# dariopagliaricci/Metal-PathTracer-arm64

Measured on AMD Instinct MI355X. Metric: Msamples/sec (whole node) at 1920×1080, depth 8; PFM RMSE vs Embree ref, higher is better.
Workload: dtype f32; 1 GPU; BASELINE configs[1]: Cornell box + one 70,688-triangle OBJ mesh, 1920x1080, depth 8, 256 spp, seed 1337; partition=8-row bands round-robin over 1 rank(s), RCCL gather of the HDR buffer

## Files before the change

### metal-pathtracer-arm64_amd/__init__.py

```python
from __future__ import annotations

import ctypes as C
import os
from typing import Optional, Tuple

import numpy as np

_PKG_DIR = os.path.dirname(os.path.abspath(__file__))
LIB_PATH = os.path.join(_PKG_DIR, "libptr_hip.so")
CLI_PATH = os.path.join(_PKG_DIR, "PathTracerHeadless")



class PtrSphere(C.Structure):
    _fields_ = [("centerRadius", C.c_float * 4), ("materialIndex", C.c_uint32 * 4)]


class PtrRect(C.Structure):
    _fields_ = [
        ("corner", C.c_float * 4),
        ("edgeU", C.c_float * 4),
        ("edgeV", C.c_float * 4),
        ("normalAndPlane", C.c_float * 4),
        ("materialTwoSided", C.c_uint32 * 4),
# ... 346 lines not shown
class PtrFrameInfo(C.Structure):
    _fields_ = [
        ("width", C.c_uint32),
        ("height", C.c_uint32),
        ("minCount", C.c_uint32),
        ("maxCount", C.c_uint32),
        ("totalSamples", C.c_uint64),
        ("uniform", C.c_uint32),
        ("reserved", C.c_uint32),
    ]


_frame_info = C.POINTER(PtrFrameInfo)
_FRAME_SIGNATURES = {
    "ptr_frame_create": (_int, [_vp, _settings, C.POINTER(_vp)] + _err),
    "ptr_frame_release": (None, [_vp]),
    "ptr_frame_reset": (_int, [_vp, _settings] + _err),
    "ptr_frame_accumulate": (_int, [_vp, _u32, _vp, _stats] + _err),
    "ptr_frame_refine": (_int, [_vp, _adaptive, _vp, _stats, _adaptive_info] + _err),
    "ptr_frame_resolve_device": (_int, [_vp, _vp, _vp, _vp, _vp] + _err),
    "ptr_frame_resolve": (_int, [_vp, _fp, _fp, _up] + _err),
    "ptr_frame_info": (_int, [_vp, _frame_info]),
    "ptr_frame_export": (_int, [_vp, _fp, _fp, _fp, _up, _fp] + _err),
    "ptr_frame_import": (_int, [_vp, _fp, _fp, _fp, _up, _fp] + _err),
    "ptr_frame_debug_create": (_int, [_u32, _u32, _fp, _u32, _int, C.POINTER(_vp)] + _err),
}
FRAME_SYMBOLS = tuple(_FRAME_SIGNATURES)

_MULTI_FRAME_SIGNATURES = {
    "ptr_multi_frame_create": (_int, [_desc, _settings, _int, C.POINTER(_vp)] + _err),
    "ptr_multi_frame_release": (None, [_vp]),
    "ptr_multi_frame_reset": (_int, [_vp, _settings] + _err),
    "ptr_multi_frame_accumulate": (_int, [_vp, _u32, _stats] + _err),
    "ptr_multi_frame_refine": (_int, [_vp, _adaptive, _stats, _adaptive_info] + _err),
    "ptr_multi_frame_resolve": (_int, [_vp, _fp, _fp, _up, _fp, _fp] + _err),
    "ptr_multi_frame_resolve_device": (_int, [_vp, _vp, _vp, _vp, _vp] + _err),
    "ptr_multi_frame_info": (_int, [_vp, _frame_info, _multi_info]),
    "ptr_multi_frame_export": (_int, [_vp, _fp, _fp, _fp, _up, _fp] + _err),
    "ptr_multi_frame_import": (_int, [_vp, _fp, _fp, _fp, _up, _fp] + _err),
    "ptr_multi_frame_debug_create_on": (_int, [_desc, _settings, _ids, _int, C.POINTER(_vp)] + _err),
    "ptr_multi_frame_debug_create": (_int, [_u32, _u32, _fp, _u32, _ids, _int, C.POINTER(_vp)] + _err),
}
MULTI_FRAME_SYMBOLS = tuple(_MULTI_FRAME_SIGNATURES)



class PtrMeshTransform(C.Structure):
    _fields_ = [("meshIndex", C.c_uint32), ("pad", C.c_uint32), ("localToWorld", C.c_float * 16)]


class PtrUpdateInfo(C.Structure):
    _fields_ = [
        ("totalSeconds", C.c_double),
        ("bakeMs", C.c_double),
        ("refitMs", C.c_double),
        ("quantiseMs", C.c_double),
        ("wideMs", C.c_double),
        ("trianglesMoved", C.c_uint64),
        ("nodes", C.c_uint64),
        ("levels", C.c_uint64),
        ("wideNodes", C.c_uint64),
        ("sceneLo", C.c_float * 3),
        ("sceneHi", C.c_float * 3),
        ("gridOrigin", C.c_float * 3),
        ("gridCell", C.c_float * 3),
        ("cellOverExtent", C.c_float),
        ("pad", C.c_uint32),
    ]

    def as_dict(self) -> dict:
        return {name: (list(getattr(self, name)) if hasattr(getattr(self, name), "__len__") else getattr(self, name))
                for name, _ in self._fields_ if name != "pad"}


_DYNAMIC_SIGNATURES = {
    "ptr_scene_upload_dynamic": (_int, [_desc, _int, C.POINTER(_vp)] + _err),
    "ptr_scene_set_mesh_transforms": (_int, [_vp, C.POINTER(PtrMeshTransform), _u32, _vp, C.POINTER(PtrUpdateInfo)] + _err),
    "ptr_scene_is_dynamic": (_int, [_vp]),
    "ptr_debug_scene_arrays": (_int, [_vp, _u32, _vp, _u64, _u64p]),
    "ptr_debug_dynamic_tables": (_int, [_desc, _u32, _vp, _u64, _u64p] + _err),
}
DYNAMIC_SYMBOLS = tuple(_DYNAMIC_SIGNATURES)

SCENE_ARRAYS = {"tris": (0, np.float32, (3, 4)), "triNormals": (1, np.float32, (3, 4)), "triUv": (2, np.float32, (4, 4)),
                "triTangent": (3, np.float32, (3, 4)), "triBounds": (4, np.float32, (2, 4)), "sphereBounds": (5, np.float32, (2, 4)),
                "boxes": (6, np.float32, (4, 4)), "qnodes": (7, np.uint32, (2, 4)), "wnodes": (8, np.uint32, (4, 4)), "grid": (9, np.float32, (3,))}
DYNAMIC_TABLES = {"nodes": (0, np.float32, (4, 4)), "qnodes": (1, np.uint32, (2, 4)), "wnodes": (2, np.uint32, (4, 4)),
                  "triBounds": (3, np.float32, (2, 4)), "sphereBounds": (4, np.float32, (2, 4)), "schedule": (5, np.uint32, ()),
                  "levelOffsets": (6, np.uint32, ()), "wideSource": (7, np.uint32, (4,)), "grid": (8, np.float32, (3,)),
                  "requantised": (9, np.uint32, (2, 4)), "meshTriOffsets": (10, np.uint32, ()), "meshTris": (11, np.uint32, ()),
                  "info": (12, np.uint32, ())}
DYNAMIC_TABLE_INFO = ("nodes", "levels", "wide_nodes", "quantized", "triangles", "spheres", "max_depth", "root_ref", "oversize_ref", "wide_depth")

_lib: Optional[C.CDLL] = None


class PtrError(RuntimeError):
    pass


def load_library() -> C.CDLL:
    global _lib
    if _lib is not None:
        return _lib
    path = os.environ.get("PTR_HIP_LIBRARY", LIB_PATH)
    if not os.path.exists(path):
        raise PtrError(f"{path} is missing: run `python -c 'import __graft_entry__ as g; g.build()'` first")
    lib = C.CDLL(path)
    for name, (restype, argtypes) in list(_SIGNATURES.items()) + list(_POST_SIGNATURES.items()) + list(_STATS_SIGNATURES.items()) + \
            list(_ADAPTIVE_SIGNATURES.items()) + list(_MULTI_SIGNATURES.items()) + list(_FRAME_SIGNATURES.items()) + list(_MULTI_FRAME_SIGNATURES.items()) + \
            list(_DYNAMIC_SIGNATURES.items()):
        fn = getattr(lib, name)
        fn.restype, fn.argtypes = restype, argtypes
    _lib = lib
    return lib


def _err_buf():
    return C.create_string_buffer(1024)


def _check(rc: int, err) -> None:
    if rc != 0:
        raise PtrError(err.value.decode("utf-8", "replace") or f"libptr_hip call failed ({rc})")


def _fptr(a: np.ndarray):
    return a.ctypes.data_as(C.POINTER(C.c_float))


def _uptr(a: np.ndarray):
    return a.ctypes.data_as(C.POINTER(C.c_uint32))


def _batch(fn, lead, inp, dtype, cols, outs, more=(), tail=()):
    ptr = lambda a: _uptr(a) if a.dtype == np.uint32 else _fptr(a)
    inp = np.ascontiguousarray(inp, dtype=dtype).reshape(-1, cols)
    res = [np.zeros((inp.shape[0],) + shape, dtype=dt) for shape, dt in outs]
    err = _err_buf()
    _check(fn(*lead, ptr(inp), *more, inp.shape[0], *map(ptr, res), *tail, err, len(err)), err)
    return res[0] if len(res) == 1 else tuple(res)


def device_count() -> int:
    return int(load_library().ptr_device_count())


BAND_ROWS = 8


def band_count(height: int, part: int = 0, parts: int = 1) -> int:
    return int(load_library().ptr_part_band_count(height, part, parts))




class HostScene:

    def __init__(self, handle: C.c_void_p):
        self._h = handle
        self.desc = PtrSceneDesc()
        self.settings = PtrSettings()
        load_library().ptr_host_scene_desc(self._h, C.byref(self.desc), C.byref(self.settings))

    @classmethod
    def load(cls, scene_path: str, asset_dir: Optional[str] = None) -> "HostScene":
        lib = load_library()
        h = C.c_void_p()
        err = _err_buf()
        rc = lib.ptr_host_scene_load(os.fsencode(scene_path), os.fsencode(asset_dir) if asset_dir else None,
                                     C.byref(h), err, len(err))
        _check(rc, err)
        return cls(h)

    def settings_for(self, width: Optional[int] = None, height: Optional[int] = None, max_depth: Optional[int] = None,
                     seed: Optional[int] = None, **overrides) -> PtrSettings:
        s = self.settings.copy()
        if width:
            s.width = width
        if height:
            s.height = height
        if max_depth is not None:
            s.maxDepth = max_depth
        if seed is not None:
            s.seed = seed
        for k, v in overrides.items():
            setattr(s, k, v)
        if s.width == 0:
            s.width = 1280
        if s.height == 0:
            s.height = 720
        return s

    def close(self) -> None:
# ... 677 lines not shown
    err = _err_buf()
    _check(lib.ptr_host_write_exr_multilayer(os.fsencode(path), _fptr(rgb), w, h, _fptr(counts) if counts is not None else None,
                                             colorspace.encode(), err, len(err)), err)


def read_pfm(path: str) -> np.ndarray:
    lib = load_library()
    w, h = C.c_uint32(), C.c_uint32()
    if lib.ptr_host_read_pfm(os.fsencode(path), None, 0, C.byref(w), C.byref(h)) != 0:
        raise PtrError(f"cannot read PFM header: {path}")
    out = np.zeros((h.value, w.value, 3), dtype=np.float32)
    if lib.ptr_host_read_pfm(os.fsencode(path), _fptr(out), out.size, C.byref(w), C.byref(h)) != 0:
        raise PtrError(f"cannot read PFM data: {path}")
    return out




def debug_eval_bsdf(material: PtrMaterial, settings: PtrSettings, inputs: np.ndarray) -> np.ndarray:
    return _batch(load_library().ptr_debug_eval_bsdf, (C.byref(material), C.byref(settings)), inputs, np.float32, 12, [((5,), np.float32)])


def debug_sample_bsdf(material: PtrMaterial, settings: PtrSettings, inputs: np.ndarray, front: np.ndarray,
                      states: np.ndarray):
    front = np.ascontiguousarray(front, dtype=np.uint32)
    states = np.ascontiguousarray(states, dtype=np.uint32)
    return _batch(load_library().ptr_debug_sample_bsdf, (C.byref(material), C.byref(settings)), inputs, np.float32, 9,
                  [((8,), np.float32), ((), np.uint32)], more=(_uptr(front), _uptr(states)))


def debug_sample_lobes(material: PtrMaterial, settings: PtrSettings, inputs: np.ndarray, front: np.ndarray, states: np.ndarray):
    front = np.ascontiguousarray(front, dtype=np.uint32)
    states = np.ascontiguousarray(states, dtype=np.uint32)
    env_rough = C.c_float()
    out, sample, out_states = _batch(load_library().ptr_debug_sample_lobes, (C.byref(material), C.byref(settings)), inputs, np.float32, 9,
                                     [((3,), np.float32), ((8,), np.float32), ((), np.uint32)], more=(_uptr(front), _uptr(states)),
                                     tail=(C.byref(env_rough),))
    return out, sample, out_states, float(env_rough.value)


def debug_env_mips(rgba: np.ndarray):
    rgba = np.ascontiguousarray(rgba, dtype=np.float32)
    h, w = rgba.shape[0], rgba.shape[1]
    lib = load_library()
    levels = C.c_uint32(0)
    if lib.ptr_debug_env_mips(_fptr(rgba), w, h, None, 0, C.byref(levels)) != 0:
        raise PtrError("ptr_debug_env_mips failed")
    sizes = [(max(h >> l, 1), max(w >> l, 1)) for l in range(levels.value)]
    out = np.zeros(sum(a * b for a, b in sizes) * 4, dtype=np.float32)
    if lib.ptr_debug_env_mips(_fptr(rgba), w, h, _fptr(out), out.size, C.byref(levels)) != 0:
        raise PtrError("ptr_debug_env_mips failed")
    chain, at = [], 0
    for a, b in sizes:
        chain.append(out[at:at + a * b * 4].reshape(a, b, 4))
        at += a * b * 4
    return chain


def debug_camera_rays(settings: PtrSettings, xys: np.ndarray):
    return _batch(load_library().ptr_debug_camera_rays, (C.byref(settings),), xys, np.uint32, 3, [((6,), np.float32), ((), np.uint32)])


def debug_env_distribution(rgba: np.ndarray) -> dict:
    rgba = np.ascontiguousarray(rgba, dtype=np.float32)
    h, w = rgba.shape[0], rgba.shape[1]
    pdf = np.zeros((h, w), np.float32)
    ca = np.zeros((h, w), np.uint32)
    ct = np.zeros((h, w), np.float32)
    ma = np.zeros(h, np.uint32)
    mt = np.zeros(h, np.float32)
    total = C.c_float()
    rc = load_library().ptr_debug_env_distribution(_fptr(rgba), w, h, _fptr(pdf), _uptr(ca), _fptr(ct), _uptr(ma), _fptr(mt),
                                                   C.byref(total))
    if rc != 0:
        raise PtrError("environment map has no positive radiance")
    return dict(pdf=pdf, cond_alias=ca, cond_threshold=ct, marg_alias=ma, marg_threshold=mt, total=total.value)


GEOMETRY_FIELDS = ("nodes", "leaves", "triangles_referenced", "spheres_referenced", "max_depth", "max_leaf_size",
                   "unreferenced", "multiply_referenced", "box_violations", "quant_violations", "bad_refs", "triangles",
                   "spheres", "sah_cost_milli", "build_ms", "quantized_usable")


def debug_scene_geometry(desc: PtrSceneDesc, leaf_max: int = 0) -> dict:
    out = (C.c_uint64 * 16)()
    err = _err_buf()
    _check(load_library().ptr_debug_scene_geometry(C.byref(desc), leaf_max, out, err, len(err)), err)
    g = dict(zip(GEOMETRY_FIELDS, [int(v) for v in out]))
    word = g["quantized_usable"]
    g["oversize"] = (word >> 8) & 0xFF
    g["wide_nodes"] = (word >> 16) & 0xFFFFFFFF
    g["wide_depth"] = (word >> 48) & 0xFF
    g["wide_problems"] = word >> 63
    g["quantized_usable"] = word & 0xFF
    return g


def debug_dynamic_tables(desc: PtrSceneDesc, names=None) -> dict:
    lib = load_library()
    out = {}
    for name in (names or DYNAMIC_TABLES):
        which, dtype, shape = DYNAMIC_TABLES[name]
        size = C.c_uint64(0)
        err = _err_buf()
        _check(lib.ptr_debug_dynamic_tables(C.byref(desc), which, None, 0, C.byref(size), err, len(err)), err)
        buf = np.zeros(size.value // np.dtype(dtype).itemsize, dtype)
        _check(lib.ptr_debug_dynamic_tables(C.byref(desc), which, buf.ctypes.data_as(C.c_void_p), buf.nbytes, C.byref(size), err, len(err)), err)
        out[name] = buf.reshape(2, 3) if name == "grid" else buf.reshape((-1,) + shape)
    if "info" in out:
        out["info"] = dict(zip(DYNAMIC_TABLE_INFO, (int(v) for v in out["info"])))
    return out


def walk_stack_depths(desc: PtrSceneDesc, rays: np.ndarray) -> np.ndarray:
    return _batch(load_library().ptr_debug_walk_stack_depths, (C.byref(desc),), rays, np.float32, 8, [((), np.uint32)])
```

### metal-pathtracer-arm64_amd/csrc/host/debug_probes.cpp

```cpp
#include <algorithm>
#include <cmath>

#include "device_scene.h"
#include "ptr_debug.h"

using namespace ptrk;
using namespace ptrhost;

namespace {

bool checkProbeRays(const float* rays, uint64_t n, bool infiniteTmax, const char* who, char* err, size_t err_cap) {
    if (n >= (1ull << kConnectMaskShift)) {
        setErr(err, err_cap, std::string(who) + ": at most 2^27 - 1 rays");
        return false;
    }
    for (uint64_t i = 0; i < n; ++i) {
        const float tmin = rays[i * 8 + 3], tmax = rays[i * 8 + 7];
        if (tmin != 1.0e-4f || (infiniteTmax && !(std::isinf(tmax) && tmax > 0.0f))) {
            setErr(err, err_cap, std::string(who) + ": ray " + std::to_string(i) + " has tmin " + std::to_string(tmin) + " / tmax " +
                                     std::to_string(tmax) + (infiniteTmax ? "; the kernel traces from 1e-4 to infinity" : "; the kernel traces from 1e-4"));
            return false;
        }
    }
    return true;
}

void probeInfo(const PtrDeviceScene& ds, bool count, uint32_t info[4]) {
    info[0] = static_cast<uint32_t>(traversalNodeFormat(ds.view, count));
    info[1] = ds.view.stackLimit;
    info[2] = ds.view.useWide ? ds.wideDepth : 0u;
    info[3] = kLdsStackLevels;
}

LaunchConfig probeLaunchConfig(const PtrDeviceScene& ds) {
    LaunchConfig cfg = coldLaunchConfig(ds);
    cfg.feederChunk = ds.feederChunk;
    HIP_CHECK(hipMemset(cfg.workCounters, 0, 2 * sizeof(uint32_t)));
    return cfg;
}

struct BsdfProbe {
    DeviceBuffer<float4> material;
    RenderParams rp;
    BsdfProbe(const PtrMaterial& m, const PtrSettings& settings) {
        std::vector<float> rows;
        compactMaterial(m, rows);
        material.upload(reinterpret_cast<const float4*>(rows.data()), kMaterialVec4);
        fillRenderParams(settings, 1, rp);
    }
};

}

extern "C" {

int ptr_debug_render_signatures(PtrDeviceScene* scene, const PtrSettings* settings, float* out_rgb, uint32_t* out_signature, char* err,
                                size_t err_cap) {
    return deviceCall("ptr_debug_render_signatures", scene, scene && settings && out_signature, err, err_cap, [&] {
        const size_t pixels = static_cast<size_t>(settings->width) * settings->height;
        const size_t floats = static_cast<size_t>(ptr_part_band_count(settings->height, 0, 1)) * PTR_BAND_ROWS * settings->width * 3u;
        scene->outBands.ensure(floats);
        PtrRenderStats stats{};
        renderBands(*scene, *settings, 1u, 0u, 1u, scene->outBands.ptr, nullptr, 1, &stats);
        if (out_rgb) scene->outBands.download(out_rgb, pixels * 3u);
        std::vector<float4> items(pixels);
        std::vector<uint32_t> pixelOfLocal(pixels);
        scene->itemAccum.download(items.data(), pixels);
        scene->pixelOfLocal.download(pixelOfLocal.data(), pixels);
        for (size_t lp = 0; lp < pixels; ++lp) {
            uint32_t bits;
            std::memcpy(&bits, &items[lp].w, sizeof(bits));
            out_signature[pixelOfLocal[lp]] = bits;
        }
    });
}

int ptr_debug_texture_sample(PtrDeviceScene* scene, uint32_t texture, const float* in, uint64_t n, float* out, char* err, size_t err_cap) {
    return deviceCall("ptr_debug_texture_sample", scene, scene && (in || !n) && (out || !n), err, err_cap, [&] {
        if (n == 0) return;
        DeviceBuffer<float> din;
        DeviceBuffer<float4> dout;
        din.upload(in, n * 3);
        dout.ensure(n);
        launchDebugTexSample(scene->view, texture, din.ptr, n, dout.ptr, nullptr);
        dout.download(reinterpret_cast<float4*>(out), n);
    });
// ... 69 lines not shown
            HIP_CHECK(hipMemset(scene->counters.ptr, 0, sizeof(uint64_t) * kCounterSlots));
            pool.counters = scene->counters.ptr;
        }
        launchExtend(scene->view, pool, probeLaunchConfig(*scene), nullptr, count != 0, nullptr);
        HIP_CHECK(hipGetLastError());
        launchDebugHitRecords(scene->view, dRays.ptr, dHit.ptr, n, static_cast<uint32_t>(scene->info[2]), static_cast<uint32_t>(scene->info[3]),
                              dOut.ptr, nullptr);
        HIP_CHECK(hipDeviceSynchronize());
        dOut.download(out, n);
    });
}

int ptr_debug_connect_rays(PtrDeviceScene* scene, const float* rays, const uint32_t* ignore_light, uint64_t n, uint32_t records_per_slot,
                           uint32_t* occluded, uint32_t info[4], char* err, size_t err_cap) {
    const bool argsOk = scene && (rays || !n) && (occluded || !n) && info;
    if (argsOk && (records_per_slot < 1u || records_per_slot > 4u)) {
        setErr(err, err_cap, "ptr_debug_connect_rays: records_per_slot must be 1..4");
        return 1;
    }
    if (argsOk && !checkProbeRays(rays, n, false, "ptr_debug_connect_rays", err, err_cap)) return 1;
    for (uint64_t i = 0; argsOk && ignore_light && i < n; ++i) {
        if (ignore_light[i] != 0xFFFFFFFFu && ignore_light[i] >= scene->view.rectLightCount) {
            setErr(err, err_cap, "ptr_debug_connect_rays: ray " + std::to_string(i) + " ignores light " + std::to_string(ignore_light[i]) +
                                     " of " + std::to_string(scene->view.rectLightCount));
            return 1;
        }
    }
    return deviceCall("ptr_debug_connect_rays", scene, argsOk, err, err_cap, [&] {
        probeInfo(*scene, false, info);
        if (n == 0) return;
        std::vector<float4> lights(static_cast<size_t>(scene->view.rectLightCount) * kRectLightVec4);
        scene->rectLights.download(lights.data(), lights.size());
        const uint64_t slots = (n + records_per_slot - 1u) / records_per_slot;
        std::vector<float4> rec(slots * kRecSlots * 4u, make_float4(0.0f, 0.0f, 0.0f, 0.0f));
        for (uint64_t i = 0; i < n; ++i) {
            const float* r = rays + i * 8;
            const uint64_t slot = i / records_per_slot, k = i % records_per_slot;
            const uint32_t light = ignore_light ? ignore_light[i] : 0xFFFFFFFFu;
            const uint32_t kind = light == 0xFFFFFFFFu ? 0u : 3u;
            rec[(k * 4u + 0u) * slots + slot] = make_float4(r[0], r[1], r[2], r[7]);
            rec[(k * 4u + 1u) * slots + slot] = make_float4(r[4], r[5], r[6], bitsToFloat(kind));
            rec[(k * 4u + 2u) * slots + slot] = make_float4(1.0f, 1.0f, 1.0f, 0.0f);
            if (kind == 3u) rec[(k * 4u + 3u) * slots + slot] = make_float4(lights[static_cast<size_t>(light) * kRectLightVec4 + 6u].w, 0.0f, 0.0f, 0.0f);
        }
        std::vector<std::vector<uint32_t>> queues(kConnectQueues);
        for (uint64_t slot = 0; slot < slots; ++slot) {
            uint32_t q = static_cast<uint32_t>(((slot * 2654435761ull) >> 7) % 97u) % kConnectQueues;
            if (q % 5u == 2u) q = (q * 3u + 1u) % kConnectQueues;
            if (q % 5u == 2u) q = (q + 1u) % kConnectQueues;
            const uint32_t records = static_cast<uint32_t>(std::min<uint64_t>(records_per_slot, n - slot * records_per_slot));
            queues[q].push_back(static_cast<uint32_t>(slot) | (((1u << records) - 1u) << kConnectMaskShift));
        }
        size_t region = 1;
        for (const auto& q : queues) region = std::max(region, q.size());
        std::vector<uint32_t> list(region * kConnectQueues, 0u), counts(kConnectQueues * kConnectCountStride, 0u);
        for (uint32_t q = 0; q < kConnectQueues; ++q) {
            std::copy(queues[q].begin(), queues[q].end(), list.begin() + static_cast<size_t>(q) * region);
            counts[q * kConnectCountStride] = static_cast<uint32_t>(queues[q].size());
        }
        DeviceBuffer<float4> dRec;
        DeviceBuffer<uint32_t> dList, dCounts;
        dRec.upload(rec.data(), rec.size());
        dList.upload(list.data(), list.size());
        dCounts.upload(counts.data(), counts.size());
        PathPool pool{};
        for (uint32_t k = 0; k < kRecSlots; ++k) {
            pool.rec[k] = ShadowRecordView{dRec.ptr + (k * 4u + 0u) * slots, dRec.ptr + (k * 4u + 1u) * slots, dRec.ptr + (k * 4u + 2u) * slots,
                                           dRec.ptr + (k * 4u + 3u) * slots};
        }
        pool.slots = static_cast<uint32_t>(slots);
        pool.recStride = static_cast<uint32_t>(slots);
        pool.connectList = dList.ptr;
        pool.connectCount = dCounts.ptr;
        pool.connectRegion = static_cast<uint32_t>(region);
        RenderParams rp{};
        launchConnect(rp, scene->view, pool, probeLaunchConfig(*scene), false, nullptr);
        HIP_CHECK(hipDeviceSynchronize());
        dRec.download(rec.data(), rec.size());
        for (uint64_t i = 0; i < n; ++i) {
            const float4 a = rec[((i % records_per_slot) * 4u + 2u) * slots + i / records_per_slot];
            occluded[i] = (a.x == 0.0f && a.y == 0.0f && a.z == 0.0f) ? 1u : 0u;
        }
    });
}

int ptr_debug_exact_division(uint32_t d, const uint32_t* n, uint64_t count, uint32_t* out) {
    if (d == 0u || (!n && count) || (!out && count)) return 1;
    const DivU32 by = makeDivU32(d);
    for (uint64_t i = 0; i < count; ++i) out[i] = by.quotient(n[i]);
    return 0;
}

int ptr_debug_shade_kernel_set(const PtrDeviceScene* scene, const PtrSettings* settings, int count, uint32_t* out) {
    if (!scene || !settings || !out) return 1;
    RenderParams rp;
    fillRenderParams(*settings, 1, rp);
    *out = shadeKernelSet(rp, scene->view, count != 0);
    return 0;
}

int ptr_debug_eval_bsdf(const PtrMaterial* material, const PtrSettings* settings, const float* in, uint64_t n, float* out,
                        char* err, size_t err_cap) {
    return deviceCall("ptr_debug_eval_bsdf", nullptr, material && settings && (in || !n) && (out || !n), err, err_cap, [&] {
        BsdfProbe probe(*material, *settings);
        DeviceBuffer<float> din, dout;
        din.upload(in, n * 12);
        dout.ensure(n * 5);
        launchDebugEvalBsdf(probe.material.ptr, probe.rp, din.ptr, n, dout.ptr, nullptr);
        dout.download(out, n * 5);
    });
}

int ptr_debug_sample_bsdf(const PtrMaterial* material, const PtrSettings* settings, const float* in, const uint32_t* front_face,
                          const uint32_t* rng_states, uint64_t n, float* out, uint32_t* out_states, char* err, size_t err_cap) {
    const bool argsOk = material && settings && ((in && front_face && rng_states && out && out_states) || !n);
    return deviceCall("ptr_debug_sample_bsdf", nullptr, argsOk, err, err_cap, [&] {
        BsdfProbe probe(*material, *settings);
        DeviceBuffer<float> din, dout;
        DeviceBuffer<uint32_t> dfront, drng, drngOut;
        din.upload(in, n * 9);
        dfront.upload(front_face, n);
        drng.upload(rng_states, n);
        dout.ensure(n * 8);
        drngOut.ensure(n);
        launchDebugSampleBsdf(probe.material.ptr, probe.rp, din.ptr, dfront.ptr, drng.ptr, n, dout.ptr, drngOut.ptr, nullptr);
        dout.download(out, n * 8);
        drngOut.download(out_states, n);
    });
}

int ptr_debug_sample_lobes(const PtrMaterial* material, const PtrSettings* settings, const float* in, const uint32_t* front_face,
                           const uint32_t* rng_states, uint64_t n, float* out, float* out_sample, uint32_t* out_states, float* env_roughness,
                           char* err, size_t err_cap) {
    const bool argsOk = material && settings && ((in && front_face && rng_states) || !n);
    return deviceCall("ptr_debug_sample_lobes", nullptr, argsOk, err, err_cap, [&] {
        BsdfProbe probe(*material, *settings);
        DeviceBuffer<float> din, dout, dsample;
        DeviceBuffer<uint32_t> dfront, drng, drngOut;
        din.upload(in, n * 9);
        dfront.upload(front_face, n);
        drng.upload(rng_states, n);
        dout.ensure(n * 3 + 1);
        dsample.ensure(n * 8);
        drngOut.ensure(n);
        if (n > 0) {
            launchDebugSampleLobes(probe.material.ptr, probe.rp, din.ptr, dfront.ptr, drng.ptr, n, dout.ptr, dsample.ptr, drngOut.ptr, nullptr);
        } else {
            HIP_CHECK(hipMemset(dout.ptr, 0, sizeof(float)));
        }
        std::vector<float> o(n * 3 + 1, 0.0f);
        dout.download(o.data(), o.size());
        if (out) std::memcpy(out, o.data(), n * 3 * sizeof(float));
        if (env_roughness) *env_roughness = o[n * 3];
        if (out_sample) dsample.download(out_sample, n * 8);
        if (out_states) drngOut.download(out_states, n);
    });
}

int ptr_debug_env_lookup(PtrDeviceScene* scene, const PtrSettings* settings, const float* in, uint64_t n, float* out, char* err, size_t err_cap) {
    return deviceCall("ptr_debug_env_lookup", scene, scene && settings && (in || !n) && (out || !n), err, err_cap, [&] {
        if (scene->view.envWidth == 0u) throw HipError{"ptr_debug_env_lookup: the scene has no environment map"};
        ensureEnvMips(*scene);
        if (n == 0) return;
        RenderParams rp;
        fillRenderParams(*settings, 1, rp);
        const EnvLodView env{scene->envMips.ptr, nullptr, scene->envMipLevels, 0u};
// ... 134 lines not shown
```

### metal-pathtracer-arm64_amd/csrc/host/device_scene.h

```cpp
#pragma once

#include <hip/hip_runtime.h>

#include <cstdio>
#include <cstring>
#include <exception>
#include <functional>
#include <memory>
#include <string>
#include <vector>

#include "../kernels/device_types.h"
#include "../kernels/launch.h"
#include "env_importance_sampler.h"
#include "geometry_cache.h"
#include "ptr_abi.h"

namespace ptrhost {

struct HipError {
    std::string message;
};

#define HIP_CHECK(expr)                                                                                     \
    do {                                                                                                    \
        hipError_t _e = (expr);                                                                             \
        if (_e != hipSuccess) {                                                                             \
            throw ptrhost::HipError{std::string(#expr) + ": " + hipGetErrorString(_e)};                     \
        }                                                                                                   \
    } while (0)

inline void setErr(char* err, size_t cap, const std::string& msg) {
    if (err && cap > 0) std::snprintf(err, cap, "%s", msg.c_str());
}

#define PTR_CATCH_ALL(err, cap)                                                                             \
    catch (const ptrhost::HipError& e) {                                                                    \
        ptrhost::setErr(err, cap, e.message);                                                               \
        return 1;                                                                                           \
    }                                                                                                       \
    catch (const std::exception& e) {                                                                       \
        ptrhost::setErr(err, cap, std::string("exception: ") + e.what());                                   \
        return 1;                                                                                           \
    }                                                                                                       \
    catch (...) {                                                                                           \
        ptrhost::setErr(err, cap, "unknown exception");                                                     \
        return 1;                                                                                           \
    }

template <typename T>
struct DeviceBuffer {
    T* ptr = nullptr;
    size_t count = 0;
    DeviceBuffer() = default;
    DeviceBuffer(const DeviceBuffer&) = delete;
    DeviceBuffer& operator=(const DeviceBuffer&) = delete;
    ~DeviceBuffer() { release(); }
    void release() {
        if (ptr) (void)hipFree(ptr);
        ptr = nullptr;
        count = 0;
    }
    void ensure(size_t n) {
        if (n <= count && ptr) return;
        release();
        if (n == 0) n = 1;
        HIP_CHECK(hipMalloc(reinterpret_cast<void**>(&ptr), n * sizeof(T)));
        count = n;
    }
    void upload(const T* src, size_t n) {
        ensure(n);
        if (n) HIP_CHECK(hipMemcpy(ptr, src, n * sizeof(T), hipMemcpyHostToDevice));
    }
    void download(T* dst, size_t n) const {
        if (n) HIP_CHECK(hipMemcpy(dst, ptr, n * sizeof(T), hipMemcpyDeviceToHost));
    }
};

inline float bitsToFloat(uint32_t u) {
    float f;
    std::memcpy(&f, &u, 4);
    return f;
}

}

#include "adaptive_state.h"

using ptrhost::DeviceBuffer;

namespace ptrhost {

struct DynamicScene {
    DeviceBuffer<float4> objPos, objNrm, objTan;
    DeviceBuffer<float4> triBounds, sphereBounds;
    DeviceBuffer<float4> boxes;
    DeviceBuffer<uint32_t> meshTris, schedule, wideSource;
    DeviceBuffer<float4> meshTable;
    std::vector<uint32_t> meshTriOffsets, levelOffsets;
    std::vector<uint8_t> meshHasTangents;
    uint32_t nodeCount = 0, wideCount = 0, triCount = 0, sphereCount = 0;
    bool textured = false;
    float meanPrimExtent = 0.0f;
    hipEvent_t events[5] = {nullptr, nullptr, nullptr, nullptr, nullptr};
    float4* rootBox = nullptr;
    ~DynamicScene() {
        for (hipEvent_t e : events) {
            if (e) (void)hipEventDestroy(e);
        }
        if (rootBox) (void)hipHostFree(rootBox);
    }
};

}

struct PtrDeviceScene {
    int device = 0;
    DeviceBuffer<uint4> qnodes;
    DeviceBuffer<uint4> wnodes;
    DeviceBuffer<float4> nodes, tris, triNormals, spheres, materials, rects, rectLights, envRgba;
    DeviceBuffer<uint2> sphereInfo;
    DeviceBuffer<int32_t> lightIndexByRect;
    DeviceBuffer<float2> envCond, envMarg, cone;
    DeviceBuffer<float4> triUv, triTangent, texels, materialTex;
    DeviceBuffer<uint4> texInfo;
    DeviceBuffer<float> envPdf;
    DeviceBuffer<float4> envMips;
    uint32_t envMipLevels = 0;
    ptrk::SceneView view{};
    std::unique_ptr<ptrhost::DynamicScene> dynamic;
    uint64_t info[8] = {0};
    double uploadSeconds = 0.0;
    double timings[4] = {0.0, 0.0, 0.0, 0.0};
    uint64_t deviceTotalBytes = 0;
    bool hasRandomWalkMaterial = false;

    DeviceBuffer<float4> state, recBuf, itemAccum;
    DeviceBuffer<float2> hit;
    DeviceBuffer<uint32_t> flushItem, signature, tailList, tailWords;
    DeviceBuffer<uint32_t> connectList, connectCounts;
    DeviceBuffer<uint32_t> busyLists, busyCounts;
    uint64_t tailBelow = 512ull << 10;
    uint64_t poolSlots = 32ull << 20;
    uint32_t poolGroups = 0;
    bool connectOverlap = true;
    uint32_t maxPoolGroups() const { return poolGroups ? poolGroups : 4u; }
    uint32_t feederChunk = 256;
    std::vector<hipStream_t> groupStreams;
    std::vector<hipEvent_t> groupEvents;
    std::vector<hipStream_t> sideStreams;
    std::vector<hipEvent_t> sideEvents;
    int refillBelow = 40;
    uint32_t spillLevels = 0;
    uint32_t wideDepth = 0;
    DeviceBuffer<uint4> medium;
    DeviceBuffer<float> envLod;
    DeviceBuffer<uint32_t> scalars, pixelOfLocal, spill;
    DeviceBuffer<uint2> itemReserve;
    DeviceBuffer<uint32_t> itemHeads, zeros;
    DeviceBuffer<uint64_t> counters;
    DeviceBuffer<float> outBands;
    DeviceBuffer<float> covBands;
    DeviceBuffer<float4> covMean;
    ptrhost::AdaptiveStore adaptive;
    DeviceBuffer<float> adaptiveOut;
    DeviceBuffer<float4> rayBatch;
    DeviceBuffer<PtrHit> hitBatch;
    uint32_t* pinnedAlive = nullptr;
    uint32_t traceGrid = 0;
    uint32_t traceGridHalf = 0;
    uint32_t cachedW = 0, cachedH = 0, cachedPart = 0, cachedParts = 0, cachedLocalPixels = 0;

    ~PtrDeviceScene() {
        if (pinnedAlive) (void)hipHostFree(pinnedAlive);
        for (hipStream_t st : groupStreams) (void)hipStreamDestroy(st);
        for (hipEvent_t e : groupEvents) (void)hipEventDestroy(e);
        for (hipStream_t st : sideStreams) (void)hipStreamDestroy(st);
        for (hipEvent_t e : sideEvents) (void)hipEventDestroy(e);
    }
};

namespace ptrhost {

void compactMaterial(const PtrMaterial& m, std::vector<float>& out);
void appendTextureWithMips(const PtrTexture& t, std::vector<float>& texels, std::vector<uint32_t>& info);
double ensureEnvMips(PtrDeviceScene& ds);
void fillRenderParams(const PtrSettings& s, uint32_t spp, ptrk::RenderParams& rp);
ptrk::LaunchConfig coldLaunchConfig(const PtrDeviceScene& ds);
void renderBands(PtrDeviceScene& ds, const PtrSettings& settings, uint32_t spp, uint32_t part, uint32_t parts, float* dOut, hipStream_t stream,
                 int mode, PtrRenderStats* stats, float* dCov = nullptr);
uint32_t framePasses(const PtrDeviceScene& ds, const PtrSettings& settings, uint32_t spp);

uint64_t maxPassItems(const PtrDeviceScene* ds);
void traceItems(PtrDeviceScene& ds, const PtrSettings& settings, uint32_t spp, uint32_t sampleBase, const uint32_t* dPixelOfLocal,
                uint32_t localPixels, hipStream_t stream, PtrRenderStats* stats, const std::function<void(const float4*)>& consume);
void imagePixelOrder(uint32_t width, uint32_t height, std::vector<uint32_t>& out);
void addPassStats(const PtrRenderStats& one, PtrRenderStats& sum);
void addLaunchStats(PtrRenderStats& a, const PtrRenderStats& b);

void partitionPixels(uint32_t width, uint32_t height, uint32_t part, uint32_t parts, std::vector<uint32_t>& out);
struct PreparedScene {
    ptr::PreparedGeometry pg;
    std::vector<float> mats, lights;
    std::vector<int32_t> lightIndexByRect;
    uint32_t lightCount = 0;
    bool lightsHaveTriangles = true;
    bool hasRandomWalkMaterial = false;
    ptr::EnvImportanceDistribution envDist;
    bool hasEnvDist = false;
    std::vector<float> texels;
    std::vector<uint32_t> texInfo;
    std::vector<float> materialTex;
    double geometrySeconds = 0.0;
    double shadingSeconds = 0.0;
    bool geometryFromCache = false;
    double seconds = 0.0;
    bool dynamic = false;
    ptr::DynamicTables dyn;
};
void prepareGeometry(const PtrSceneDesc& desc, ptr::PreparedGeometry& pg, ptr::DynamicTables* dyn = nullptr);
void prepareScene(const PtrSceneDesc& desc, PreparedScene& ps, const char* cachePath = nullptr, bool dynamic = false);
void uploadScene(const PtrSceneDesc& desc, const PreparedScene& ps, PtrDeviceScene& ds);
void uploadDynamicTables(const PreparedScene& ps, PtrDeviceScene& ds);

inline int refuse(char* err, size_t cap, const std::string& message) {
    setErr(err, cap, message);
    return 1;
}
inline int nullArgument(const char* who, char* err, size_t cap) { return refuse(err, cap, std::string(who) + ": null argument"); }
inline int noDevice(const char* who, char* err, size_t cap) {
    setErr(err, cap, std::string(who) + ": no HIP device (the HIP path has no CPU fallback)");
    return 2;
}
constexpr uint64_t kIndexLimit = 0xFFFF0000ull;
inline bool pastIndexLimit(uint64_t count) { return count > kIndexLimit; }

template <typename Body>
int deviceCall(const char* who, const PtrDeviceScene* scene, bool argsOk, char* err, size_t cap, Body&& body) {
    if (!argsOk) return nullArgument(who, err, cap);
    try {
        if (!scene && ptr_device_count() < 1) throw HipError{"no HIP device (the HIP path has no CPU fallback)"};
        HIP_CHECK(hipSetDevice(scene ? scene->device : 0));
        body();
        HIP_CHECK(hipGetLastError());
        return 0;
    }
    PTR_CATCH_ALL(err, cap)
}

}
```

### metal-pathtracer-arm64_amd/csrc/host/dynamic.cpp

```cpp
#include <algorithm>
#include <chrono>
#include <cmath>

#include "../kernels/bvh_grid.h"
#include "../kernels/dynamic.h"
#include "device_scene.h"
#include "ptr_dynamic.h"

using namespace ptrk;
using namespace ptrhost;

namespace ptrhost {

void uploadDynamicTables(const PreparedScene& ps, PtrDeviceScene& ds) {
    const ptr::DynamicTables& t = ps.dyn;
    const ptr::FlatBvh& bvh = ps.pg.geo.bvh;
    auto dyn = std::make_unique<DynamicScene>();
    dyn->objPos.upload(reinterpret_cast<const float4*>(t.objPos.data()), t.objPos.size() / 4);
    dyn->objNrm.upload(reinterpret_cast<const float4*>(t.objNrm.data()), t.objNrm.size() / 4);
    dyn->textured = ds.view.triUv != nullptr;
    if (dyn->textured) dyn->objTan.upload(reinterpret_cast<const float4*>(t.objTan.data()), t.objTan.size() / 4);
    dyn->triBounds.upload(reinterpret_cast<const float4*>(t.triBounds.data()), t.triBounds.size() / 4);
    dyn->sphereBounds.upload(reinterpret_cast<const float4*>(t.sphereBounds.data()), t.sphereBounds.size() / 4);
    if (ps.pg.useQuantized) dyn->boxes.upload(reinterpret_cast<const float4*>(bvh.nodes.data()), bvh.nodes.size() / 4);
// ... 43 lines not shown
    if (bake.det3 == 0.0f || !std::isfinite(bake.det3)) return "has a zero 3x3 determinant";
    for (int a = 0; a < 3; ++a) {
        if (!std::isfinite(bake.nc0[a]) || !std::isfinite(bake.nc1[a]) || !std::isfinite(bake.nc2[a])) return "has a cofactor inverse that is not finite";
    }
    return "";
}

}

extern "C" {

int ptr_scene_is_dynamic(const PtrDeviceScene* scene) { return scene && scene->dynamic ? 1 : 0; }

int ptr_scene_set_mesh_transforms(PtrDeviceScene* scene, const PtrMeshTransform* transforms, uint32_t count, void* stream, PtrUpdateInfo* info,
                                  char* err, size_t err_cap) {
    const char* who = "ptr_scene_set_mesh_transforms";
    if (!scene) return nullArgument(who, err, err_cap);
    if (!scene->dynamic) return refuse(err, err_cap, std::string(who) + ": the scene is not dynamic (upload it with ptr_scene_upload_dynamic)");
    if (!transforms) return refuse(err, err_cap, std::string(who) + ": null transform list");
    if (count == 0u) return refuse(err, err_cap, std::string(who) + ": count is 0");
    DynamicScene& dyn = *scene->dynamic;
    const uint32_t meshCount = static_cast<uint32_t>(dyn.meshTriOffsets.size()) - 1u;
    std::vector<DynMeshRow> rows(count);
    try {
        std::vector<uint8_t> named(meshCount, 0);
        for (uint32_t i = 0; i < count; ++i) {
            const PtrMeshTransform& t = transforms[i];
            if (t.meshIndex >= meshCount) {
                return refuse(err, err_cap, std::string(who) + ": mesh index " + std::to_string(t.meshIndex) + " out of range (the scene has " +
                                                std::to_string(meshCount) + " meshes)");
            }
            if (named[t.meshIndex]++) return refuse(err, err_cap, std::string(who) + ": mesh index " + std::to_string(t.meshIndex) + " named twice");
            ptr::MeshBake bake;
            ptr::ComputeMeshBake(t.localToWorld, bake);
            const std::string problem = matrixProblem(t.localToWorld, bake);
            if (!problem.empty()) return refuse(err, err_cap, std::string(who) + ": the matrix of mesh " + std::to_string(t.meshIndex) + " " + problem);
            DynMeshRow& r = rows[i];
            std::memset(&r, 0, sizeof(r));
            std::memcpy(r.l2w, bake.localToWorld, sizeof(r.l2w));
            std::memcpy(r.nc0, bake.nc0, 12);
            std::memcpy(r.nc1, bake.nc1, 12);
            std::memcpy(r.nc2, bake.nc2, 12);
            r.detSign = bake.detSign;
            r.hasTangents = dyn.meshHasTangents[t.meshIndex] ? 1.0f : 0.0f;
        }
    }
    PTR_CATCH_ALL(err, err_cap)

    return deviceCall(who, scene, true, err, err_cap, [&] {
        const auto t0 = std::chrono::steady_clock::now();
        hipStream_t st = static_cast<hipStream_t>(stream);
        PtrDeviceScene& ds = *scene;
        SceneView& v = ds.view;
        dyn.meshTable.ensure(static_cast<size_t>(count) * kDynMeshVec4);
        HIP_CHECK(hipMemcpyAsync(dyn.meshTable.ptr, rows.data(), rows.size() * sizeof(DynMeshRow), hipMemcpyHostToDevice, st));
        HIP_CHECK(hipEventRecord(dyn.events[0], st));
        DynBakeArrays arrays{dyn.objPos.ptr, dyn.objNrm.ptr, dyn.textured ? dyn.objTan.ptr : nullptr, ds.tris.ptr, ds.triNormals.ptr, dyn.triBounds.ptr,
                             dyn.textured ? ds.triUv.ptr : nullptr, dyn.textured ? ds.triTangent.ptr : nullptr};
        uint64_t moved = 0;
        for (uint32_t i = 0; i < count; ++i) {
            const uint32_t m = transforms[i].meshIndex;
            const uint32_t first = dyn.meshTriOffsets[m], n = dyn.meshTriOffsets[m + 1u] - first;
            launchDynBake(arrays, dyn.meshTable.ptr, i, dyn.meshTris.ptr + first, n, st);
            moved += n;
        }
        HIP_CHECK(hipEventRecord(dyn.events[1], st));
        float4* boxes = floatBoxes(ds);
        const uint32_t levels = static_cast<uint32_t>(dyn.levelOffsets.size()) - 1u;
        for (uint32_t l = 0; l < levels; ++l) {
            launchDynRefitLevel(boxes, dyn.schedule.ptr + dyn.levelOffsets[l], dyn.levelOffsets[l + 1u] - dyn.levelOffsets[l], dyn.triBounds.ptr,
                                dyn.sphereBounds.ptr, st);
        }
        HIP_CHECK(hipEventRecord(dyn.events[2], st));
        float lo[3] = {0, 0, 0}, hi[3] = {0, 0, 0};
        if (dyn.nodeCount > 0u) {
            HIP_CHECK(hipMemcpyAsync(dyn.rootBox, boxes, 4 * sizeof(float4), hipMemcpyDeviceToHost, st));
            HIP_CHECK(hipStreamSynchronize(st));
            if (rootBoxOf(dyn.rootBox, lo, hi)) {
                for (int a = 0; a < 3; ++a) {
                    gridAxis(lo[a], hi[a], v.gridOrigin[a], v.gridCell[a]);
                    v.gridInvCell[a] = 1.0f / v.gridCell[a];
                }
            }
        }
        if (v.useQuantized) launchDynQuantise(boxes, ds.qnodes.ptr, dyn.nodeCount, v.gridOrigin, v.gridCell, st);
        HIP_CHECK(hipEventRecord(dyn.events[3], st));
        if (v.useWide) launchDynWide(ds.qnodes.ptr, ds.wnodes.ptr, dyn.wideSource.ptr, dyn.wideCount * 4u, st);
        HIP_CHECK(hipEventRecord(dyn.events[4], st));
        HIP_CHECK(hipStreamSynchronize(st));
        if (info) {
            std::memset(info, 0, sizeof(*info));
            float ms[4] = {0, 0, 0, 0};
            for (int g = 0; g < 4; ++g) HIP_CHECK(hipEventElapsedTime(&ms[g], dyn.events[g], dyn.events[g + 1]));
            info->bakeMs = ms[0], info->refitMs = ms[1], info->quantiseMs = ms[2], info->wideMs = ms[3];
            info->trianglesMoved = moved;
            info->nodes = dyn.nodeCount;
            info->levels = levels;
            info->wideNodes = dyn.wideCount;
            for (int a = 0; a < 3; ++a) {
                info->sceneLo[a] = lo[a], info->sceneHi[a] = hi[a];
                info->gridOrigin[a] = v.gridOrigin[a], info->gridCell[a] = v.gridCell[a];
            }
            const float maxCell = std::max(std::max(v.gridCell[0], v.gridCell[1]), v.gridCell[2]);
            info->cellOverExtent = dyn.meanPrimExtent > 0.0f ? maxCell / dyn.meanPrimExtent : 0.0f;
            info->totalSeconds = std::chrono::duration<double>(std::chrono::steady_clock::now() - t0).count();
        }
    });
}

int ptr_debug_scene_arrays(PtrDeviceScene* scene, uint32_t which, void* out, uint64_t cap_bytes, uint64_t* size_out) {
    if (!scene || !size_out) return 1;
    const PtrDeviceScene& ds = *scene;
    const DynamicScene* dyn = ds.dynamic.get();
    const uint64_t tris = ds.info[2], spheres = ds.info[3], nodes = ds.info[0];
    const void* src = nullptr;
    uint64_t bytes = 0;
    switch (which) {
        case PTR_SCENE_ARRAY_TRIS: src = ds.tris.ptr, bytes = tris * 48u; break;
        case PTR_SCENE_ARRAY_TRI_NORMALS: src = ds.triNormals.ptr, bytes = tris * 48u; break;
        case PTR_SCENE_ARRAY_TRI_UV: src = ds.triUv.ptr, bytes = ds.view.triUv ? tris * 64u : 0u; break;
        case PTR_SCENE_ARRAY_TRI_TANGENT: src = ds.triTangent.ptr, bytes = ds.view.triTangent ? tris * 48u : 0u; break;
        case PTR_SCENE_ARRAY_TRI_BOUNDS: src = dyn ? dyn->triBounds.ptr : nullptr, bytes = dyn ? tris * 32u : 0u; break;
        case PTR_SCENE_ARRAY_SPHERE_BOUNDS: src = dyn ? dyn->sphereBounds.ptr : nullptr, bytes = dyn ? spheres * 32u : 0u; break;
        case PTR_SCENE_ARRAY_BOXES:
            src = ds.view.useQuantized ? (dyn ? dyn->boxes.ptr : nullptr) : ds.nodes.ptr;
            bytes = src ? nodes * 64u : 0u;
            break;
        case PTR_SCENE_ARRAY_QNODES: src = ds.qnodes.ptr, bytes = ds.view.useQuantized ? nodes * 32u : 0u; break;
        case PTR_SCENE_ARRAY_WNODES: src = ds.wnodes.ptr, bytes = ds.view.useWide ? ds.view.wideBytes : 0u; break;
        case PTR_SCENE_ARRAY_GRID: bytes = 24u; break;
        default: return 1;
    }
    *size_out = bytes;
    if (!out) return 0;
    if (cap_bytes < bytes) return 2;
    if (bytes == 0u) return 0;
    if (which == PTR_SCENE_ARRAY_GRID) {
        std::memcpy(out, ds.view.gridOrigin, 12);
        std::memcpy(static_cast<char*>(out) + 12, ds.view.gridCell, 12);
        return 0;
    }
    if (hipSetDevice(ds.device) != hipSuccess || hipMemcpy(out, src, bytes, hipMemcpyDeviceToHost) != hipSuccess) return 3;
    return 0;
}

int ptr_debug_dynamic_tables(const PtrSceneDesc* scene, uint32_t which, void* out, uint64_t cap_bytes, uint64_t* size_out, char* err, size_t err_cap) {
    if (!scene || !size_out) return nullArgument("ptr_debug_dynamic_tables", err, err_cap);
    try {
        ptr::PreparedGeometry pg;
        ptr::DynamicTables t;
        prepareGeometry(*scene, pg, &t);
        const ptr::FlatBvh& bvh = pg.geo.bvh;
        std::vector<uint32_t> words;
        const void* src = nullptr;
        uint64_t bytes = 0;
        auto take = [&](const void* p, size_t n) { src = p, bytes = n; };
        switch (which) {
            case PTR_DYNAMIC_TABLE_NODES: take(bvh.nodes.data(), bvh.nodes.size() * 4u); break;
            case PTR_DYNAMIC_TABLE_QNODES: take(bvh.qnodes.data(), bvh.qnodes.size() * 4u); break;
            case PTR_DYNAMIC_TABLE_WNODES: take(pg.wide.get(), static_cast<size_t>(pg.wideCount) * 64u); break;
            case PTR_DYNAMIC_TABLE_TRI_BOUNDS: take(t.triBounds.data(), t.triBounds.size() * 4u); break;
            case PTR_DYNAMIC_TABLE_SPHERE_BOUNDS: take(t.sphereBounds.data(), t.sphereBounds.size() * 4u); break;
            case PTR_DYNAMIC_TABLE_SCHEDULE: take(t.schedule.data(), t.schedule.size() * 4u); break;
            case PTR_DYNAMIC_TABLE_LEVEL_OFFSETS: take(t.levelOffsets.data(), t.levelOffsets.size() * 4u); break;
            case PTR_DYNAMIC_TABLE_WIDE_SOURCE: take(t.wideSource.data(), pg.wideCount > 0u ? t.wideSource.size() * 4u : 0u); break;
            case PTR_DYNAMIC_TABLE_GRID:
// ... 37 lines not shown
```

### metal-pathtracer-arm64_amd/csrc/host/hip_backend.cpp

```cpp
#include <hip/hip_runtime.h>

#include <algorithm>
#include <chrono>
#include <cmath>
#include <cstdio>
#include <cstdlib>
#include <cstring>
#include <exception>
#include <memory>
#include <string>
#include <functional>
#include <vector>

#include "bvh_builder.h"
#include "device_scene.h"
#include "env_importance_sampler.h"
#include "geometry_cache.h"
#include "knobs.h"
#include "ptr_dynamic.h"
#include "scene_geometry.h"
#include "vecmath.h"

using namespace ptrk;
using namespace ptrhost;
// ... 184 lines not shown
    if (useQuantized) {
        ds.nodes.release();
        ds.qnodes.upload(reinterpret_cast<const uint4*>(bvh.qnodes.data()), bvh.qnodes.size() / 4);
    } else {
        ds.qnodes.release();
        ds.nodes.upload(reinterpret_cast<const float4*>(bvh.nodes.data()), bvh.nodes.size() / 4);
    }
    ds.tris.upload(reinterpret_cast<const float4*>(geo.triData.data()), geo.triData.size() / 4);
    ds.triNormals.upload(reinterpret_cast<const float4*>(geo.triNormals.data()), geo.triNormals.size() / 4);
    ds.spheres.upload(reinterpret_cast<const float4*>(geo.sphereData.data()), geo.sphereData.size() / 4);
    ds.sphereInfo.upload(reinterpret_cast<const uint2*>(geo.sphereInfo.data()), geo.sphereInfo.size() / 2);
    ds.materials.upload(reinterpret_cast<const float4*>(ps.mats.data()), ps.mats.size() / 4);
    ds.rects.upload(reinterpret_cast<const float4*>(desc.rects), static_cast<size_t>(desc.rectCount) * 5);
    ds.rectLights.upload(reinterpret_cast<const float4*>(ps.lights.data()), ps.lights.size() / 4);
    ds.lightIndexByRect.upload(ps.lightIndexByRect.data(), ps.lightIndexByRect.size());

    SceneView& v = ds.view;
    std::memset(&v, 0, sizeof(v));
    v.nodes = ds.nodes.ptr;
    v.tris = ds.tris.ptr;
    v.triNormals = ds.triNormals.ptr;
    v.spheres = ds.spheres.ptr;
    v.sphereInfo = ds.sphereInfo.ptr;
    v.materials = ds.materials.ptr;
    v.rects = ds.rects.ptr;
    v.rectLights = ds.rectLights.ptr;
    v.lightIndexByRect = ds.lightIndexByRect.ptr;
    v.qnodes = ds.qnodes.ptr;
    std::memcpy(v.gridOrigin, bvh.gridOrigin, sizeof(v.gridOrigin));
    std::memcpy(v.gridCell, bvh.gridCell, sizeof(v.gridCell));
    for (int a = 0; a < 3; ++a) v.gridInvCell[a] = 1.0f / bvh.gridCell[a];
    v.useQuantized = useQuantized ? 1u : 0u;
    if (ps.pg.wideCount > 0u) {
        ds.wnodes.upload(reinterpret_cast<const uint4*>(ps.pg.wide.get()), static_cast<size_t>(ps.pg.wideCount) * 4u);
        v.wnodes = ds.wnodes.ptr;
        v.wideBytes = static_cast<uint32_t>(static_cast<size_t>(ps.pg.wideCount) * 64u);
        v.useWide = 1u;
    }
    const size_t nodeBytes = v.useQuantized ? bvh.qnodes.size() * 4u : bvh.nodes.size() * 4u;
    const size_t triBytes = geo.triData.size() * 4u;
    if (nodeBytes > 0xFFFFFFFFull || triBytes > 0xFFFFFFFFull) throw HipError{"scene exceeds the 4 GiB node/triangle array limit"};
    v.nodeBytes = static_cast<uint32_t>(nodeBytes);
    v.triBytes = static_cast<uint32_t>(triBytes);
    v.rootRef = bvh.rootRef;
    v.oversizeRef = bvh.oversizeRef;
    v.materialCount = desc.materialCount;
    v.rectCount = desc.rectCount;
    v.rectLightCount = lightCount;
    for (uint32_t i = 0; i < desc.materialCount; ++i) v.materialTypes |= 1u << std::min(static_cast<uint32_t>(desc.materials[i].typeEta[0]), 7u);
    v.settleRectLights = (lightCount > 0u && lightCount <= kSettleLightsMax && ps.lightsHaveTriangles) ? 1u : 0u;

    if (desc.envRgba && desc.envWidth > 0 && desc.envHeight > 0) {
        const size_t texels = static_cast<size_t>(desc.envWidth) * desc.envHeight;
        ds.envRgba.upload(reinterpret_cast<const float4*>(desc.envRgba), texels);
        v.envRgba = ds.envRgba.ptr;
        v.envWidth = desc.envWidth;
        v.envHeight = desc.envHeight;
        if (ps.hasEnvDist) {
            const ptr::EnvImportanceDistribution& dist = ps.envDist;
            static_assert(sizeof(ptr::AliasEntry) == sizeof(float2), "alias entry layout");
            ds.envCond.upload(reinterpret_cast<const float2*>(dist.conditional.data()), dist.conditional.size());
            ds.envMarg.upload(reinterpret_cast<const float2*>(dist.marginal.data()), dist.marginal.size());
            ds.envPdf.upload(dist.texelPdf.data(), dist.texelPdf.size());
            v.envCond = ds.envCond.ptr;
            v.envMarg = ds.envMarg.ptr;
            v.envPdf = ds.envPdf.ptr;
            v.envSampling = 1u;
        }
    }

    if (!ps.texels.empty()) {
        ds.triUv.upload(reinterpret_cast<const float4*>(geo.triUv.data()), geo.triUv.size() / 4);
        ds.triTangent.upload(reinterpret_cast<const float4*>(geo.triTangent.data()), geo.triTangent.size() / 4);
        ds.texels.upload(reinterpret_cast<const float4*>(ps.texels.data()), ps.texels.size() / 4);
        ds.texInfo.upload(reinterpret_cast<const uint4*>(ps.texInfo.data()), ps.texInfo.size() / 4);
        ds.materialTex.upload(reinterpret_cast<const float4*>(ps.materialTex.data()), ps.materialTex.size() / 4);
        v.triUv = ds.triUv.ptr;
        v.triTangent = ds.triTangent.ptr;
        v.texels = ds.texels.ptr;
        v.texInfo = ds.texInfo.ptr;
        v.materialTex = ds.materialTex.ptr;
        v.textureCount = desc.textureCount;
    }

    if (ps.dynamic) uploadDynamicTables(ps, ds);

    ds.info[0] = bvh.nodeCount;
    ds.info[1] = bvh.leafCount;
    ds.info[2] = triCount;
    ds.info[3] = desc.sphereCount;
    ds.info[4] = bvh.maxDepth;
    ds.info[5] = bvh.maxLeafSize;
    ds.info[6] = static_cast<uint64_t>(bvh.sahCost * 1000.0);
    ds.info[7] = lightCount;

    hipDeviceProp_t prop;
    HIP_CHECK(hipGetDeviceProperties(&prop, ds.device));
    ds.deviceTotalBytes = prop.totalGlobalMem;
    const uint32_t cus = prop.multiProcessorCount > 0 ? static_cast<uint32_t>(prop.multiProcessorCount) : 256u;
    ds.traceGrid = cus * 8u;
    if (knobs.refillBelow > 0) ds.refillBelow = knobs.refillBelow;
    ds.traceGridHalf = cus * 4u;
    if (knobs.tailBelow >= 0) ds.tailBelow = static_cast<uint64_t>(knobs.tailBelow);
    if (knobs.poolSlots != 0) ds.poolSlots = knobs.poolSlots;
    if (knobs.poolGroups != 0) ds.poolGroups = knobs.poolGroups;
    ds.connectOverlap = knobs.connectOverlap != 0;
    const uint32_t wideLevels = ps.pg.wideCount > 0u ? ps.pg.wideDepth : 0u;
    const uint32_t stackNeed = std::min<uint32_t>(kTraversalStackDepth, std::max(3u * wideLevels, static_cast<uint32_t>(bvh.maxDepth)) + 4u);
    v.stackLimit = std::max(stackNeed, kLdsStackLevels);
    ds.wideDepth = wideLevels;
    ds.spillLevels = v.stackLimit - kLdsStackLevels;
    ds.spill.ensure(std::max<size_t>(spillWordsPerGroup(ds) * ds.maxPoolGroups() * 2u, 1u));
    ds.scalars.ensure(static_cast<size_t>(kScalarCount) * kMaxPoolGroups);
    ds.counters.ensure(kCounterSlots);
    ds.zeros.ensure(16);
    HIP_CHECK(hipMemset(ds.zeros.ptr, 0, 16 * sizeof(uint32_t)));
    HIP_CHECK(hipHostMalloc(reinterpret_cast<void**>(&ds.pinnedAlive), sizeof(uint32_t) * (kPinnedHeadsOffset + kItemHeads), hipHostMallocDefault));
    const double copySeconds = std::chrono::duration<double>(std::chrono::steady_clock::now() - t0).count();
    ds.uploadSeconds = ps.seconds + copySeconds;
    ds.timings[0] = ps.geometrySeconds;
    ds.timings[1] = ps.shadingSeconds;
    ds.timings[2] = copySeconds;
    ds.timings[3] = ps.geometryFromCache ? 1.0 : 0.0;
    if (knobs.verboseBuild) std::fprintf(stderr, "[upload] prepare %.2f s, copies to the device %.2f s\n", ps.seconds, copySeconds);
}

}

namespace {

int uploadTo(const char* who, const PtrSceneDesc* scene, const char* cachePath, int device, PtrDeviceScene** outScene, char* err, size_t cap,
             bool dynamic = false) {
    if (!scene || !outScene) return nullArgument(who, err, cap);
    if (ptr_device_count() <= device || device < 0) {
        setErr(err, cap, std::string(who) + ": no such HIP device (the HIP path has no CPU fallback)");
        return 2;
    }
    try {
        auto ds = std::make_unique<PtrDeviceScene>();
        ds->device = device;
        PreparedScene ps;
        prepareScene(*scene, ps, cachePath, dynamic);
        uploadScene(*scene, ps, *ds);
        *outScene = ds.release();
        return 0;
    }
    PTR_CATCH_ALL(err, cap)
}

void buildCamera(const PtrSettings& s, CameraParams& c) {
    constexpr float kPiF = 3.14159265358979323846f;
    const float aspect = s.width > 0 ? static_cast<float>(s.width) / static_cast<float>(s.height) : 1.0f;
    const float vfov = std::min(std::max(s.cameraVerticalFov, 1.0f), 179.0f);
    const float defocus = std::max(s.cameraDefocusAngle, 0.0f);
    const float theta = vfov * (kPiF / 180.0f);
    const float h = std::tan(theta * 0.5f);
    const float viewportHeight = 2.0f * h;
    const float viewportWidth = aspect * viewportHeight;
    const float distance = std::max(s.cameraDistance, 0.1f);
    const float cp = std::cos(s.cameraPitch), sp = std::sin(s.cameraPitch);
    const float cy = std::cos(s.cameraYaw), sy = std::sin(s.cameraYaw);
    const float3 offset{distance * cp * cy, distance * sp, distance * cp * sy};
    const float3 lookAt{s.cameraTarget[0], s.cameraTarget[1], s.cameraTarget[2]};
    const float3 lookFrom = lookAt + offset;
    const float3 w = ptr::normalize(lookFrom - lookAt);
    const float3 u = ptr::normalize(ptr::cross(float3{0.0f, 1.0f, 0.0f}, w));
// ... 18 lines not shown
}

}

namespace ptrhost {

double ensureEnvMips(PtrDeviceScene& ds) {
    if (ds.envMipLevels > 0u || ds.view.envRgba == nullptr || ds.view.envWidth == 0u || ds.view.envHeight == 0u) return 0.0;
    const auto t0 = std::chrono::steady_clock::now();
    HIP_CHECK(hipSetDevice(ds.device));
    const uint32_t w = ds.view.envWidth, h = ds.view.envHeight;
    const size_t level0 = static_cast<size_t>(w) * h;
    std::vector<float> rgba(level0 * 4u);
    HIP_CHECK(hipMemcpy(rgba.data(), ds.view.envRgba, level0 * sizeof(float4), hipMemcpyDeviceToHost));
    const PtrTexture t{rgba.data(), w, h, 0u, 0u, 1u, 0u};
    std::vector<float> chain;
    std::vector<uint32_t> info;
    appendTextureWithMips(t, chain, info);
    const uint32_t levels = info[2];
    for (uint32_t l = 1; l < levels; ++l) info[4 + l] -= static_cast<uint32_t>(level0);
    static_assert(kTexInfoWords == 4u * 5u, "texture record layout");
    std::vector<float> upload(kTexInfoWords + (chain.size() - level0 * 4u));
    std::memcpy(upload.data(), info.data(), kTexInfoWords * sizeof(uint32_t));
    std::copy(chain.begin() + static_cast<std::ptrdiff_t>(level0 * 4u), chain.end(), upload.begin() + kTexInfoWords);
    ds.envMips.upload(reinterpret_cast<const float4*>(upload.data()), upload.size() / 4u);
    ds.envMipLevels = levels;
    const double ms = std::chrono::duration<double, std::milli>(std::chrono::steady_clock::now() - t0).count();
    if (ptr::readKnobs().verboseBuild) std::fprintf(stderr, "[upload] environment mip chain: %ux%u, %u levels, %.2f ms\n", w, h, levels, ms);
    return ms;
}

void fillRenderParams(const PtrSettings& s, uint32_t spp, RenderParams& rp) {
    std::memset(&rp, 0, sizeof(rp));
    buildCamera(s, rp.cam);
    rp.width = s.width;
    rp.byWidth = makeDivU32(s.width);
    rp.height = s.height;
    rp.maxDepth = std::min(s.maxDepth, kFlagFieldMask);
    rp.shadowSlack = (s.debugShadowSlack > 0.0f && s.debugShadowSlack < 1.0f) ? s.debugShadowSlack : 0.0f;
    rp.seedBase = s.seed != 0 ? s.seed : 0x9e3779b9u;
    rp.spp = std::max(1u, spp);
    rp.sampleBase = 0u;
    rp.sppTotal = rp.spp;
    rp.passFlags = 3u;
    rp.enableRussianRoulette = s.enableRussianRoulette;
    rp.enableSpecularNee = s.enableSpecularNee;
    rp.enableMnee = s.enableMnee;
    rp.enableMneeSecondary = s.enableMneeSecondary;
    rp.backgroundMode = s.backgroundMode;
    std::memcpy(rp.backgroundColor, s.backgroundColor, sizeof(rp.backgroundColor));
    rp.envRotation = s.environmentRotation;
    rp.envIntensity = s.environmentIntensity;
    rp.clampFactor = std::max(s.fireflyClampFactor, 0.0f);
    rp.clampFloor = std::max(s.fireflyClampFloor, 0.0f);
    rp.throughputClamp = std::max(s.throughputClamp, 0.0f);
    rp.tailClampBase = std::max(s.specularTailClampBase, 0.0f);
    rp.tailClampRoughnessScale = std::max(s.specularTailClampRoughnessScale, 0.0f);
    rp.minSpecularPdf = std::max(s.minSpecularPdf, 1.0e-8f);
    rp.clampEnabled = s.fireflyClampEnabled ? 1.0f : 0.0f;
    rp.emissionScale = (s.emissionScale > 0.0f && std::isfinite(s.emissionScale)) ? s.emissionScale : 1.0f;
    rp.mediaMode = s.metalSemantics & (PTR_METAL_MEDIA | PTR_METAL_THIN | PTR_METAL_FACE_NORMAL | PTR_METAL_SPECULAR | PTR_METAL_SSS | PTR_METAL_PBR |
                                       PTR_METAL_CLAMPS | PTR_METAL_ENV_LOD | PTR_METAL_RAY_DIFF);
    rp.clampMaxContribution = std::max(s.fireflyClampMaxContribution, 0.0f);
    rp.minSpecularPdfRaw = s.minSpecularPdf;
    rp.sssMode = s.sssMode;
    rp.sssMaxSteps = std::max(s.sssMaxSteps, 1u);
}

LaunchConfig coldLaunchConfig(const PtrDeviceScene& ds) { return LaunchConfig{ds.traceGrid, ds.spill.ptr, ds.scalars.ptr + 1, ds.refillBelow}; }

void partitionPixels(uint32_t width, uint32_t height, uint32_t part, uint32_t parts, std::vector<uint32_t>& out) {
    out.clear();
    const uint32_t bands = (height + PTR_BAND_ROWS - 1u) / PTR_BAND_ROWS;
    for (uint32_t b = part; b < bands; b += parts) {
        const uint32_t y0 = b * PTR_BAND_ROWS, y1 = std::min(y0 + PTR_BAND_ROWS, height);
        for (uint32_t ty = y0; ty < y1; ty += 8u) {
            for (uint32_t tx = 0; tx < width; tx += 8u) {
                for (uint32_t y = ty; y < std::min(ty + 8u, y1); ++y) {
                    for (uint32_t x = tx; x < std::min(tx + 8u, width); ++x) out.push_back(y * width + x);
                }
            }
        }
    }
}

void addLaunchStats(PtrRenderStats& a, const PtrRenderStats& b) {
    a.traceKernelMs += b.traceKernelMs;
    a.shadeKernelMs += b.shadeKernelMs;
    a.shadowKernelMs += b.shadowKernelMs;
    a.tailKernelMs += b.tailKernelMs;
    a.traceLaunches += b.traceLaunches;
    a.samples += b.samples;
}

}

namespace {

uint64_t itemBudgetBytes(const PtrDeviceScene& ds) {
    return std::max<uint64_t>(64ull << 20, std::min<uint64_t>(16ull << 30, ds.deviceTotalBytes / 4u));
}

bool conePaths(const PtrDeviceScene& ds, const RenderParams& rp) { return (rp.mediaMode & PTR_METAL_PBR) && ds.view.textureCount > 0u; }
bool envLodPaths(const PtrDeviceScene& ds, const RenderParams& rp) { return (rp.mediaMode & PTR_METAL_ENV_LOD) && ds.view.envWidth > 0u; }

void sizeSlots(PtrDeviceScene& ds, const RenderParams& rp, bool count, uint32_t slots) {
    ds.state.ensure(static_cast<size_t>(slots) * 4u);
    ds.hit.ensure(slots);
    ds.flushItem.ensure(slots);
    if (count) ds.signature.ensure(slots);
    if (ds.tailBelow > 0) {
        ds.tailList.ensure(slots);
        ds.tailWords.ensure(4);
    }
    ds.itemAccum.ensure(rp.itemCount);
    ds.recBuf.ensure(static_cast<size_t>(slots) * kRecSlots * 4u);
    ds.itemReserve.ensure((slots + 63u) / 64u);
    if (rp.mediaMode & PTR_METAL_MEDIA) ds.medium.ensure(slots);
    if (conePaths(ds, rp)) ds.cone.ensure(slots);
    if (envLodPaths(ds, rp)) {
        ensureEnvMips(ds);
        ds.envLod.ensure(slots);
    }
    ds.itemHeads.ensure(kItemHeadWords);
}

PathPool slotRange(const PtrDeviceScene& ds, const RenderParams& rp, bool count, uint32_t slots, uint32_t first, uint32_t n, EnvLodView& env) {
    PathPool p;
    std::memset(&p, 0, sizeof(p));
    float4* state = ds.state.ptr + first;
    p.ray0 = state;
    p.ray1 = state + slots;
    p.thr = state + 2ull * slots;
    p.accum = state + 3ull * slots;
    p.hit = ds.hit.ptr + first;
    p.flushItem = ds.flushItem.ptr + first;
    p.signature = count ? ds.signature.ptr + first : nullptr;
    p.medium = (rp.mediaMode & PTR_METAL_MEDIA) ? ds.medium.ptr + first : nullptr;
    p.cone = conePaths(ds, rp) ? ds.cone.ptr + first : nullptr;
    for (uint32_t k = 0; k < kRecSlots; ++k) {
        float4* base = ds.recBuf.ptr + static_cast<size_t>(k) * 4u * slots + first;
        p.rec[k] = ShadowRecordView{base, base + slots, base + 2ull * slots, base + 3ull * slots};
    }
    p.itemReserve = ds.itemReserve.ptr + first / 64u;
    p.slots = n;
    p.recStride = slots;
    p.itemAccum = ds.itemAccum.ptr;
    p.nextItem = ds.itemHeads.ptr;
    p.pixelOfLocal = ds.pixelOfLocal.ptr;
    p.counters = ds.counters.ptr;
    p.zero = reinterpret_cast<const float4*>(ds.zeros.ptr);
    env = EnvLodView{};
    if (envLodPaths(ds, rp)) env = EnvLodView{ds.envMips.ptr, ds.envLod.ptr + first, ds.envMipLevels, 0u};
    return p;
}

constexpr size_t kConnectCountWords = static_cast<size_t>(kConnectQueues) * kConnectCountStride;

struct PoolGroup {
    PathPool pool;
    EnvLodView env;
    LaunchConfig cfg;
    hipStream_t stream;
    hipStream_t side = nullptr;
    hipEvent_t shadeDone = nullptr, connectDone = nullptr;
    uint32_t* sideSpill = nullptr;
// ... 74 lines not shown
        gr.busyLists = ds.busyLists.ptr + connectListWords * 2u * g;
        gr.busyCounts = ds.busyCounts.ptr + kConnectCountWords * 3u * g;
        gr.scalars = ds.scalars.ptr + static_cast<size_t>(g) * kScalarCount;
        const bool sideBySide = groupCount > 1 && gr.pool.slots >= kHalfGridGroupSlots;
        gr.cfg = LaunchConfig{sideBySide ? ds.traceGridHalf : ds.traceGrid, ds.spill.ptr + g * spillWords, gr.scalars + 1, ds.refillBelow};
        gr.stream = g == 0 ? stream : ds.groupStreams[g - 1];
        gr.feederChunk = ds.feederChunk;
        if (overlap) {
            gr.side = ds.sideStreams[g];
            gr.shadeDone = ds.sideEvents[2 * g];
            gr.connectDone = ds.sideEvents[2 * g + 1];
            gr.sideSpill = ds.spill.ptr + (ds.maxPoolGroups() + g) * spillWords;
        }
    }
    return groups;
}

uint64_t itemRangeStart(const RenderParams& rp, uint32_t k) {
    return std::min<uint64_t>(static_cast<uint64_t>(rp.itemHeadFirst) + static_cast<uint64_t>(k) * rp.itemsPerHead, rp.itemCount);
}

constexpr uint64_t kPollEvery = 4;
constexpr uint64_t kPollDry = 2;

struct PollResult {
    bool allDone, runTail, queueDry;
    uint64_t nextCheck;
};

PollResult poll(PtrDeviceScene& ds, std::vector<PoolGroup>& groups, const RenderParams& rp, uint32_t slots, uint64_t iterations, bool queueDry,
                bool tracePolls) {
    HIP_CHECK(hipGetLastError());
    const uint32_t ring = static_cast<uint32_t>((iterations - 1u) % kAliveRing);
    bool headsCopied = false;
    for (uint32_t g = 0; g < groups.size(); ++g) {
        PoolGroup& gr = groups[g];
        if (gr.done) continue;
        if (queueDry) {
            HIP_CHECK(hipMemcpyAsync(ds.pinnedAlive + g, gr.scalars + kAliveBase + ring, sizeof(uint32_t), hipMemcpyDeviceToHost, gr.stream));
        } else if (!headsCopied) {
            HIP_CHECK(hipMemcpy2DAsync(ds.pinnedAlive + kPinnedHeadsOffset, sizeof(uint32_t), ds.itemHeads.ptr, sizeof(uint32_t) * kItemHeadStride,
                                       sizeof(uint32_t), kItemHeads, hipMemcpyDeviceToHost, gr.stream));
            headsCopied = true;
        }
    }
    PollResult r{true, false, queueDry, 0};
    uint64_t live = 0;
    for (uint32_t g = 0; g < groups.size(); ++g) {
        PoolGroup& gr = groups[g];
        if (gr.done) continue;
        HIP_CHECK(hipStreamSynchronize(gr.stream));
        if (queueDry) {
            if (tracePolls) {
                std::fprintf(stderr, "[poll] iteration %llu group %u live %u of %u chunk %u\n", static_cast<unsigned long long>(iterations), g,
                             ds.pinnedAlive[g], gr.pool.slots, gr.feederChunk);
            }
            gr.polledDry(ds.pinnedAlive[g], ds.feederChunk);
            if (!gr.done) live += ds.pinnedAlive[g];
        }
        r.allDone = r.allDone && gr.done;
    }
    if (queueDry && !r.allDone && ds.tailBelow > 0 && live <= ds.tailBelow) r.runTail = true;
    if (r.allDone || r.runTail) return r;
    r.nextCheck = iterations + (queueDry && ds.tailBelow > 0 ? kPollDry : kPollEvery);
    if (!queueDry) {
        uint64_t head = slots;
        const uint32_t* heads = ds.pinnedAlive + kPinnedHeadsOffset;
        for (uint32_t k = 0; k < kItemHeads; ++k) {
            const uint64_t lo = itemRangeStart(rp, k);
            const uint64_t hi = std::min<uint64_t>(lo + rp.itemsPerHead, rp.itemCount);
            head += std::min<uint64_t>(std::max<uint64_t>(heads[k], lo), hi) - lo;
        }
        if (head >= rp.itemCount) {
            r.queueDry = true;
        } else if (head > slots) {
            const double perIteration = static_cast<double>(head - slots) / static_cast<double>(iterations);
            const double left = static_cast<double>(rp.itemCount - head) / std::max(perIteration, 1.0);
            r.nextCheck = iterations + std::max<uint64_t>(kPollEvery, static_cast<uint64_t>(left * 0.75));
        }
    }
    return r;
}

enum class SpanKind : int { Extend = 0, Shade = 1, Connect = 2, Tail = 3, ResolveCov = 4 };

struct LaunchTimer {
    struct Span {
        hipEvent_t a, b;
        SpanKind kind;
        const void* stream;
    };
    bool on = false;
    std::vector<Span> spans;
    ~LaunchTimer() {
        for (const Span& s : spans) {
            for (hipEvent_t e : {s.a, s.b}) if (e) (void)hipEventDestroy(e);
        }
    }
    template <typename F>
    void launch(SpanKind kind, hipStream_t st, F&& fn) {
        if (!on) {
            fn();
            return;
        }
        spans.push_back(Span{nullptr, nullptr, kind, st});
        Span& s = spans.back();
        HIP_CHECK(hipEventCreate(&s.a));
        HIP_CHECK(hipEventCreate(&s.b));
        HIP_CHECK(hipEventRecord(s.a, st));
        fn();
        HIP_CHECK(hipEventRecord(s.b, st));
    }
};

void passStats(const PtrDeviceScene& ds, const RenderParams& rp, const std::vector<LaunchTimer::Span>& spans, bool count, const ptr::Knobs& knobs,
               double seconds, PtrRenderStats& stats) {
    std::memset(&stats, 0, sizeof(stats));
    stats.totalSeconds = seconds;
    stats.avgMsPerSample = seconds * 1000.0 / rp.spp;
    stats.uploadSeconds = ds.uploadSeconds;
    stats.samples = static_cast<uint64_t>(rp.localPixels) * rp.spp;
    if (knobs.verboseLaunches && !spans.empty()) {
        for (const LaunchTimer::Span& s : spans) {
            float t0 = 0.0f, t1 = 0.0f;
            HIP_CHECK(hipEventElapsedTime(&t0, spans.front().a, s.a));
            HIP_CHECK(hipEventElapsedTime(&t1, spans.front().a, s.b));
            std::fprintf(stderr, "[launch] kind %d  start %.3f  end %.3f  (%.3f ms)  stream %p\n", static_cast<int>(s.kind), t0, t1, t1 - t0, s.stream);
        }
    }
    for (const LaunchTimer::Span& s : spans) {
        float ms = 0.0f;
        HIP_CHECK(hipEventElapsedTime(&ms, s.a, s.b));
        switch (s.kind) {
            case SpanKind::Extend: stats.traceKernelMs += ms; ++stats.traceLaunches; break;
            case SpanKind::Shade: stats.shadeKernelMs += ms; break;
            case SpanKind::Connect: stats.shadowKernelMs += ms; break;
            case SpanKind::Tail: stats.tailKernelMs += ms; break;
            case SpanKind::ResolveCov: break;
        }
    }
    if (!count) return;
    uint64_t c[kCounterSlots];
    HIP_CHECK(hipMemcpy(c, ds.counters.ptr, sizeof(c), hipMemcpyDeviceToHost));
    stats.primaryRays = c[kCntPrimaryRays];
    stats.extendRays = c[kCntExtendRays];
    stats.shadowRays = c[kCntShadowRays];
    stats.extendNodesVisited = c[kCntExtendNodes];
    stats.extendLeafPrimTests = c[kCntExtendPrims];
    stats.nodesVisited = c[kCntExtendNodes] + c[kCntShadowNodes];
    stats.leafPrimTests = c[kCntExtendPrims] + c[kCntShadowPrims];
    stats.shadedHits = c[kCntShadedHits];
    stats.triangleHits = c[kCntTriangleHits];
    stats.shadowEarlyExits = c[kCntShadowEarlyExit];
    if (!knobs.verboseSteps) return;
    const double nodeLanes = static_cast<double>(c[kCntExtendNodes] - c[kCntExtendLeaves]), primLanes = static_cast<double>(c[kCntExtendPrims]);
    const double nodeSlots = static_cast<double>(c[kCntExtendWaveNodeSteps]), primSlots = static_cast<double>(c[kCntExtendWavePrimSteps]);
    std::fprintf(stderr, "[steps] k_extend: %.3g rays; node steps %.3g lane / %.3g slots = %.3f; prim steps %.3g lane / %.3g slots = %.3f; "
                         "refill passes %.3g (x64 lanes)\n",
                 static_cast<double>(c[kCntExtendRays]), nodeLanes, nodeSlots, nodeLanes / std::max(nodeSlots, 1.0), primLanes, primSlots,
                 primLanes / std::max(primSlots, 1.0), static_cast<double>(c[kCntExtendRefillPasses]));
    const double votes = static_cast<double>(c[kCntExtendVoteIterations]) / 64.0;
    std::fprintf(stderr, "[steps] k_extend: %.3g vote iterations; lanes holding a ray %.1f / 64 on average, of which at a leaf %.1f\n", votes,
                 static_cast<double>(c[kCntExtendActiveLanes]) / std::max(votes, 1.0), static_cast<double>(c[kCntExtendLeafLanes]) / std::max(votes, 1.0));
    const double shadeLanes = std::max(static_cast<double>(c[kCntShadeWaves]), 1.0);
    std::fprintf(stderr, "[steps] k_shade: %.3g wave visits; share of their lanes at each stage: ray traced %.3f, surface hit %.3f, of which a light "
                         "%.3f; light sample evaluated %.3f, tested against the light's own triangles %.3f, shadow ray queued %.3f; BSDF sampled "
                         "%.3f; new work item wanted %.3f\n",
                 shadeLanes / 64.0, c[kCntShadeAlive] / shadeLanes, c[kCntShadeSurface] / shadeLanes, c[kCntShadeEmitter] / shadeLanes,
                 c[kCntShadeLightEval] / shadeLanes, c[kCntShadeLightPretest] / shadeLanes, c[kCntShadeLightStored] / shadeLanes,
                 c[kCntShadeBsdfSample] / shadeLanes, c[kCntShadeNeedItem] / shadeLanes);
    static const char* names[kShadeParts] = {"loads + landing", "background", "surface reconstruction", "emitter", "light sample", "env sample",
                                             "BSDF sample + next ray", "work item + camera ray", "stores + lists", "subsurface walk"};
    double waveTotal = 0.0;
    for (uint32_t k = 0; k < kShadeParts; ++k) waveTotal += static_cast<double>(c[kCntShadeWaveTicks + k]);
    std::fprintf(stderr, "[steps] k_shade parts (clock ticks between the part's first and last instruction, waits included): share of the waves' time | lanes busy\n");
    for (uint32_t k = 0; k < kShadeParts; ++k) {
        const double wave = static_cast<double>(c[kCntShadeWaveTicks + k]), lane = static_cast<double>(c[kCntShadeLaneTicks + k]);
        if (wave <= 0.0) continue;
        std::fprintf(stderr, "[steps]   %-24s %5.1f %% | %.3f\n", names[k], 100.0 * wave / std::max(waveTotal, 1.0), lane / (64.0 * wave));
    }
    std::fprintf(stderr, "[steps] k_extend: refill passes take %.1f %% of the waves' time in the kernel\n",
                 100.0 * static_cast<double>(c[kCntExtendRefillTicks]) / std::max(static_cast<double>(c[kCntExtendWaveTicks]), 1.0));
}

template <typename Resolve>
void tracePass(PtrDeviceScene& ds, const PtrSettings& settings, uint32_t spp, uint32_t sampleBase, uint32_t sppTotal, uint32_t passFlags,
               const uint32_t* dPixelOfLocal, uint32_t localPixels, hipStream_t stream, int mode, PtrRenderStats* stats, Resolve&& resolve);

void renderPass(PtrDeviceScene& ds, const PtrSettings& settings, uint32_t spp, uint32_t sampleBase, uint32_t sppTotal, uint32_t passFlags,
                uint32_t part, uint32_t parts, float* dOut, float* dCov, hipStream_t stream, int mode, PtrRenderStats* stats) {
    if (ds.cachedW != settings.width || ds.cachedH != settings.height || ds.cachedPart != part || ds.cachedParts != parts) {
        std::vector<uint32_t> pixels;
        partitionPixels(settings.width, settings.height, part, parts, pixels);
        ds.pixelOfLocal.upload(pixels.data(), pixels.size());
        ds.cachedW = settings.width;
        ds.cachedH = settings.height;
        ds.cachedPart = part;
        ds.cachedParts = parts;
        ds.cachedLocalPixels = static_cast<uint32_t>(pixels.size());
    }
    const uint32_t localPixels = ds.cachedLocalPixels;
    const uint32_t bandCount = ptr_part_band_count(settings.height, part, parts);
    const size_t outFloats = static_cast<size_t>(bandCount) * PTR_BAND_ROWS * settings.width * 3u;
    if (passFlags & 1u) HIP_CHECK(hipMemsetAsync(dOut, 0, outFloats * sizeof(float), stream));
    if (dCov && (passFlags & 1u)) HIP_CHECK(hipMemsetAsync(dCov, 0, outFloats * 2u * sizeof(float), stream));
    if (localPixels == 0) {
        HIP_CHECK(hipStreamSynchronize(stream));
        return;
    }
    tracePass(ds, settings, spp, sampleBase, sppTotal, passFlags, ds.pixelOfLocal.ptr, localPixels, stream, mode, stats,
              [&](const RenderParams& rp, const PathPool& pool, LaunchTimer& timer) {
                  launchResolve(rp, pool, parts, dOut, stream);
                  if (dCov) {
                      ds.covMean.ensure(localPixels);
                      timer.launch(SpanKind::ResolveCov, stream, [&] { launchResolveCov(rp, pool, parts, ds.covMean.ptr, dCov, stream); });
                  }
              });
}

template <typename Resolve>
void tracePass(PtrDeviceScene& ds, const PtrSettings& settings, uint32_t spp, uint32_t sampleBase, uint32_t sppTotal, uint32_t passFlags,
               const uint32_t* dPixelOfLocal, uint32_t localPixels, hipStream_t stream, int mode, PtrRenderStats* stats, Resolve&& resolve) {
    const bool count = (mode & 1) != 0;
    const bool soloGroup = (mode & 2) != 0;

    RenderParams rp;
    fillRenderParams(settings, spp, rp);
    rp.sampleBase = sampleBase;
    rp.sppTotal = std::max(1u, sppTotal);
    rp.passFlags = passFlags;

    rp.localPixels = localPixels;
    rp.byLocalPixels = makeDivU32(localPixels);
    const uint64_t itemCount64 = static_cast<uint64_t>(localPixels) * rp.spp;
    if (itemCount64 > 0xFFFF0000ull) throw HipError{"too many work items for one pass (reduce spp or resolution)"};
    rp.itemCount = static_cast<uint32_t>(itemCount64);
    const uint64_t targetSlots = std::min<uint64_t>(ds.poolSlots, std::max<uint64_t>(1ull << 20, itemCount64 / 2u));
    uint32_t slots = static_cast<uint32_t>(std::min<uint64_t>(targetSlots, itemCount64));
    if (slots < itemCount64) slots &= ~255u;
    rp.itemHeadFirst = slots;
    rp.itemsPerHead = static_cast<uint32_t>(((itemCount64 - slots + kItemHeads - 1u) / kItemHeads + 63u) & ~63ull);

    sizeSlots(ds, rp, count, slots);
    EnvLodView env;
    PathPool pool = slotRange(ds, rp, count, slots, 0u, slots, env);
    pool.pixelOfLocal = dPixelOfLocal;
    std::vector<PoolGroup> groups = makeGroups(ds, rp, count, soloGroup, slots, stream);
    for (PoolGroup& gr : groups) gr.pool.pixelOfLocal = dPixelOfLocal;
    LaunchTimer timer{stats != nullptr};

    if (count && (passFlags & 1u)) HIP_CHECK(hipMemsetAsync(ds.counters.ptr, 0, sizeof(uint64_t) * kCounterSlots, stream));
    HIP_CHECK(hipMemsetAsync(ds.scalars.ptr, 0, sizeof(uint32_t) * kScalarCount * kMaxPoolGroups, stream));
    HIP_CHECK(hipMemsetAsync(ds.connectCounts.ptr, 0, sizeof(uint32_t) * kConnectCountWords * 2u * kMaxPoolGroups, stream));
    HIP_CHECK(hipMemsetAsync(ds.busyCounts.ptr, 0, sizeof(uint32_t) * kConnectCountWords * 3u * kMaxPoolGroups, stream));
    uint32_t* heads = ds.pinnedAlive + kPinnedHeadsOffset;
    for (uint32_t k = 0; k < kItemHeads; ++k) heads[k] = static_cast<uint32_t>(itemRangeStart(rp, k));
    HIP_CHECK(hipMemsetAsync(pool.nextItem, 0, sizeof(uint32_t) * kItemHeadWords, stream));
    HIP_CHECK(hipMemcpy2DAsync(pool.nextItem, sizeof(uint32_t) * kItemHeadStride, heads, sizeof(uint32_t), sizeof(uint32_t), kItemHeads,
                               hipMemcpyHostToDevice, stream));
    HIP_CHECK(hipStreamSynchronize(stream));
    HIP_CHECK(hipMemsetAsync(ds.itemReserve.ptr, 0, sizeof(uint2) * ((slots + 63u) / 64u), stream));
    if (rp.maxDepth == 0) HIP_CHECK(hipMemsetAsync(ds.itemAccum.ptr, 0, sizeof(float4) * rp.itemCount, stream));

    const auto wall0 = std::chrono::steady_clock::now();
    launchGenerate(rp, pool, stream);
    HIP_CHECK(hipGetLastError());
    HIP_CHECK(hipEventRecord(ds.groupEvents[0], stream));
    for (size_t g = 1; g < groups.size(); ++g) HIP_CHECK(hipStreamWaitEvent(groups[g].stream, ds.groupEvents[0], 0));
    uint64_t iterations = 0;
    const uint64_t perBounce = ((rp.mediaMode & PTR_METAL_SSS) && rp.sssMode == 2u && ds.hasRandomWalkMaterial) ? 1ull + rp.sssMaxSteps : 1ull;
    const uint64_t maxIterations = static_cast<uint64_t>(rp.maxDepth) * perBounce * ((itemCount64 + slots - 1) / slots + 1) + 8;
    const ptr::Knobs knobs = ptr::readKnobs();
    PollResult last{false, false, false, kPollEvery};
    while (rp.maxDepth > 0) {
        const uint32_t ring = static_cast<uint32_t>(iterations % kAliveRing);
        const bool queueDry = last.queueDry;
        for (PoolGroup& gr : groups) {
            if (gr.done) continue;
            uint32_t* aliveSlot = gr.scalars + kAliveBase + ring;
            gr.cfg.feederChunk = gr.feederChunk;
            const ShadeResets resets{gr.scalars + 1, gr.scalars + 2, gr.scalars + kAliveBase + (ring + 1u) % kAliveRing,
                                     (queueDry && gr.feederChunk > ds.feederChunk) ? 1u : 0u};
            gr.selectLists(iterations, queueDry);
            timer.launch(SpanKind::Extend, gr.stream, [&] { launchExtend(ds.view, gr.pool, gr.cfg, queueDry ? aliveSlot : nullptr, count, gr.stream); });
            PathPool shadePool = gr.pool;
            if (!gr.shadeListed) shadePool.busyIn = nullptr;
            if (gr.side && iterations > 0) HIP_CHECK(hipStreamWaitEvent(gr.stream, gr.connectDone, 0));
            timer.launch(SpanKind::Shade, gr.stream, [&] { launchShade(rp, ds.view, shadePool, resets, gr.env, count, gr.stream); });
            if (gr.side) {
                HIP_CHECK(hipEventRecord(gr.shadeDone, gr.stream));
                HIP_CHECK(hipStreamWaitEvent(gr.side, gr.shadeDone, 0));
                LaunchConfig ccfg = gr.cfg;
                ccfg.spill = gr.sideSpill;
                timer.launch(SpanKind::Connect, gr.side, [&] { launchConnect(rp, ds.view, gr.pool, ccfg, count, gr.side); });
                HIP_CHECK(hipEventRecord(gr.connectDone, gr.side));
            } else {
                timer.launch(SpanKind::Connect, gr.stream, [&] { launchConnect(rp, ds.view, gr.pool, gr.cfg, count, gr.stream); });
            }
        }
        ++iterations;
        if (iterations >= last.nextCheck || iterations >= maxIterations) {
            last = poll(ds, groups, rp, slots, iterations, last.queueDry, knobs.verbosePolls);
            if (last.allDone || last.runTail) break;
            if (iterations >= maxIterations) throw HipError{"wavefront loop did not terminate"};
        }
    }
    for (const PoolGroup& gr : groups) if (gr.side) HIP_CHECK(hipStreamWaitEvent(gr.stream, gr.connectDone, 0));
    for (size_t g = 1; g < groups.size(); ++g) {
        HIP_CHECK(hipEventRecord(ds.groupEvents[g], groups[g].stream));
        HIP_CHECK(hipStreamWaitEvent(stream, ds.groupEvents[g], 0));
    }
    if (last.runTail) {
        HIP_CHECK(hipMemsetAsync(ds.tailWords.ptr, 0, 4 * sizeof(uint32_t), stream));
        timer.launch(SpanKind::Tail, stream,
                     [&] { launchTail(rp, ds.view, pool, env, groups[0].cfg, ds.tailList.ptr, ds.tailWords.ptr, ds.tailWords.ptr + 1, count, stream); });
    }
    resolve(rp, pool, timer);
    HIP_CHECK(hipGetLastError());
    HIP_CHECK(hipStreamSynchronize(stream));
    const double seconds = std::chrono::duration<double>(std::chrono::steady_clock::now() - wall0).count();
    if (stats) passStats(ds, rp, timer.spans, count, knobs, seconds, *stats);
}

}

namespace ptrhost {

uint64_t maxPassItems(const PtrDeviceScene* ds) {
    uint64_t maxItems = 0xFFFFFFF0ull;
    if (ds) maxItems = std::min<uint64_t>(itemBudgetBytes(*ds) / sizeof(float4), maxItems);
    if (const uint64_t forced = ptr::readKnobs().maxItems) maxItems = forced;
    return maxItems;
}

uint32_t framePasses(const PtrDeviceScene& ds, const PtrSettings& settings, uint32_t spp) {
    const uint64_t maxItems = maxPassItems(&ds);
    const uint64_t pixels = static_cast<uint64_t>(settings.width) * settings.height;
    const uint64_t perPixel = std::max<uint64_t>(1u, maxItems / std::max<uint64_t>(pixels, 1u));
    return static_cast<uint32_t>((std::max(1u, spp) + perPixel - 1u) / perPixel);
}

void renderBands(PtrDeviceScene& ds, const PtrSettings& settings, uint32_t spp, uint32_t part, uint32_t parts, float* dOut,
                 hipStream_t stream, int mode, PtrRenderStats* stats, float* dCov) {
    if (settings.width == 0 || settings.height == 0) throw HipError{"render size must be non-zero"};
    if (parts == 0 || part >= parts) throw HipError{"bad partition"};
    HIP_CHECK(hipSetDevice(ds.device));
    spp = std::max(1u, spp);
    const uint32_t passes = framePasses(ds, settings, spp);
    if (passes <= 1u) {
        renderPass(ds, settings, spp, 0u, spp, 3u, part, parts, dOut, dCov, stream, mode, stats);
        return;
// ... 214 lines not shown
```

### metal-pathtracer-arm64_amd/csrc/host/knobs.cpp

```cpp
#include "knobs.h"

#include <algorithm>
#include <cstdlib>
#include <cstring>

namespace ptr {

namespace {

long long numberOr(const char* name, long long fallback) {
    const char* e = std::getenv(name);
    if (!e || !*e) return fallback;
    char* end = nullptr;
    const long long v = std::strtoll(e, &end, 10);
    return end == e ? fallback : v;
}

bool hasTopic(const char* list, const char* topic) {
    if (!list) return false;
    const size_t n = std::strlen(topic);
    for (const char* p = list; *p;) {
        const char* q = std::strchr(p, ',');
        const size_t len = q ? static_cast<size_t>(q - p) : std::strlen(p);
        if ((len == n && std::strncmp(p, topic, n) == 0) || (len == 3 && std::strncmp(p, "all", 3) == 0)) return true;
        p += len + (q ? 1 : 0);
    }
    return false;
}

}

Knobs readKnobs() {
    Knobs k;
    k.poolSlots = static_cast<uint64_t>(std::min<long long>(std::max<long long>(numberOr("PTR_POOL_SLOTS", 0), 0), 64ll << 20));
    if (k.poolSlots != 0 && k.poolSlots < 1024) k.poolSlots = 1024;
    k.poolGroups = static_cast<uint32_t>(std::min<long long>(std::max<long long>(numberOr("PTR_POOL_GROUPS", 0), 0), 8));
    k.connectOverlap = static_cast<int>(numberOr("PTR_CONNECT_OVERLAP", -1));
    k.wideNodes = static_cast<int>(numberOr("PTR_WIDE_NODES", -1));
    k.quantizedNodes = static_cast<int>(numberOr("PTR_QUANTIZED_NODES", -1));
    k.tailBelow = numberOr("PTR_TAIL_BELOW", -1);
    k.maxItems = static_cast<uint64_t>(std::max<long long>(numberOr("PTR_MAX_ITEMS", 0), 0));
    if (k.maxItems != 0 && k.maxItems < 1024) k.maxItems = 1024;
    k.refillBelow = static_cast<int>(std::min<long long>(std::max<long long>(numberOr("PTR_REFILL_BELOW", 0), 0), 64));
    k.buildThreads = static_cast<uint32_t>(std::min<long long>(std::max<long long>(numberOr("PTR_BUILD_THREADS", 0), 0), 256));
    k.noOversize = numberOr("PTR_NO_OVERSIZE", 0) != 0;
    k.denoiseTiled = static_cast<int>(numberOr("PTR_DENOISE_TILED", -1));
    const char* verbose = std::getenv("PTR_VERBOSE");
    k.verboseBuild = hasTopic(verbose, "build");
    k.verbosePolls = hasTopic(verbose, "polls");
    k.verboseLaunches = hasTopic(verbose, "launches");
    k.verboseSteps = hasTopic(verbose, "steps");
    return k;
}

}
```

### metal-pathtracer-arm64_amd/csrc/host/knobs.h

```cpp
#pragma once

#include <cstdint>

namespace ptr {

struct Knobs {
    uint64_t poolSlots = 0;
    uint32_t poolGroups = 0;
    int connectOverlap = -1;
    int wideNodes = -1;
    int quantizedNodes = -1;
    int64_t tailBelow = -1;
    uint64_t maxItems = 0;
    int refillBelow = 0;
    uint32_t buildThreads = 0;
    bool noOversize = false;
    int denoiseTiled = -1;
    bool verboseBuild = false, verbosePolls = false, verboseLaunches = false, verboseSteps = false;
};

Knobs readKnobs();

}
```

### metal-pathtracer-arm64_amd/csrc/host/stats.cpp

```cpp
#include <string>
#include <vector>

#include "device_scene.h"
#include "ptr_stats.h"

using namespace ptrhost;

namespace {

std::string badArgument(const char* who, bool pointersOk, const PtrSettings* settings, uint32_t spp, uint32_t part, uint32_t parts) {
    const std::string w(who);
    if (!pointersOk) return w + ": null argument";
    if (spp < 2u) return w + ": a sample covariance needs spp >= 2";
    if (parts == 0u || part >= parts) return w + ": bad partition";
    if (settings->width == 0u || settings->height == 0u) return w + ": render size must be non-zero";
    return std::string();
}

size_t bandPixels(const PtrSettings& s, uint32_t part, uint32_t parts) {
    return static_cast<size_t>(ptr_part_band_count(s.height, part, parts)) * PTR_BAND_ROWS * s.width;
}

}

extern "C" {

int ptr_render_bands_cov_device(PtrDeviceScene* scene, const PtrSettings* settings, uint32_t spp, uint32_t part_index,
                                uint32_t part_count, void* d_out_rgb, void* d_out_cov, void* stream, int count_traversal,
                                PtrRenderStats* stats, char* err, size_t err_cap) {
    const std::string bad = badArgument("ptr_render_bands_cov_device", scene && settings && d_out_rgb && d_out_cov, settings, spp, part_index, part_count);
    if (!bad.empty()) {
        setErr(err, err_cap, bad);
        return 1;
    }
    try {
        renderBands(*scene, *settings, spp, part_index, part_count, static_cast<float*>(d_out_rgb), static_cast<hipStream_t>(stream),
                    count_traversal, stats, static_cast<float*>(d_out_cov));
        return 0;
    }
    PTR_CATCH_ALL(err, err_cap)
}

int ptr_render_bands_cov(PtrDeviceScene* scene, const PtrSettings* settings, uint32_t spp, uint32_t part_index, uint32_t part_count,
                         float* out_rgb_bands, float* out_cov_bands, int count_traversal, PtrRenderStats* stats, char* err,
                         size_t err_cap) {
    const std::string bad = badArgument("ptr_render_bands_cov", scene && settings && out_rgb_bands && out_cov_bands, settings, spp, part_index, part_count);
    if (!bad.empty()) {
        setErr(err, err_cap, bad);
        return 1;
    }
    try {
        const size_t pixels = bandPixels(*settings, part_index, part_count);
        HIP_CHECK(hipSetDevice(scene->device));
        scene->outBands.ensure(pixels * 3u);
        scene->covBands.ensure(pixels * 6u);
        renderBands(*scene, *settings, spp, part_index, part_count, scene->outBands.ptr, nullptr, count_traversal, stats, scene->covBands.ptr);
        scene->outBands.download(out_rgb_bands, pixels * 3u);
        scene->covBands.download(out_cov_bands, pixels * 6u);
        return 0;
    }
    PTR_CATCH_ALL(err, err_cap)
}

int ptr_stats_debug_samples(PtrDeviceScene* scene, const PtrSettings* settings, uint32_t spp, float* out_samples, char* err, size_t err_cap) {
    if (scene && settings && out_samples && (spp < 1u || settings->width == 0u || settings->height == 0u)) {
        setErr(err, err_cap, "ptr_stats_debug_samples: spp and the render size must be non-zero");
        return 1;
    }
    return deviceCall("ptr_stats_debug_samples", scene, scene && settings && out_samples, err, err_cap, [&] {
        if (framePasses(*scene, *settings, spp) > 1u) throw HipError{"ptr_stats_debug_samples: the frame needs more than one pass"};
        const size_t pixels = static_cast<size_t>(settings->width) * settings->height;
        scene->outBands.ensure(bandPixels(*settings, 0u, 1u) * 3u);
        renderBands(*scene, *settings, spp, 0u, 1u, scene->outBands.ptr, nullptr, 0, nullptr);
        std::vector<float4> items(pixels * spp);
        std::vector<uint32_t> pixelOfLocal(pixels);
        scene->itemAccum.download(items.data(), items.size());
        scene->pixelOfLocal.download(pixelOfLocal.data(), pixels);
        for (uint32_t c = 0; c < spp; ++c) {
            for (size_t lp = 0; lp < pixels; ++lp) {
                const float4& a = items[c * pixels + lp];
                float* o = out_samples + (c * pixels + pixelOfLocal[lp]) * 3u;
                o[0] = a.x;
                o[1] = a.y;
                o[2] = a.z;
            }
        }
    });
}

}
```

### metal-pathtracer-arm64_amd/csrc/kernels/launch.h

```cpp
#pragma once

#include <hip/hip_runtime.h>

#include "device_types.h"
#include "ptr_abi.h"

namespace ptrk {

struct LaunchConfig {
    uint32_t traceGrid;
    uint32_t* spill;
    uint32_t* workCounters;
    int refillBelow;
    uint32_t feederChunk = 256;
};

void launchGenerate(const RenderParams& rp, const PathPool& pool, hipStream_t stream);
int traversalNodeFormat(const SceneView& sc, bool count);
void launchExtend(const SceneView& sc, const PathPool& pool, const LaunchConfig& cfg, uint32_t* aliveOut, bool count, hipStream_t stream);
struct ShadeResets {
    uint32_t* extendHead;
    uint32_t* connectHead;
    uint32_t* nextAlive;
    uint32_t drained;
};
void launchShade(const RenderParams& rp, const SceneView& sc, const PathPool& pool, const ShadeResets& resets, const EnvLodView& env, bool count,
                 hipStream_t stream);
uint32_t shadeKernelSet(const RenderParams& rp, const SceneView& sc, bool count);
void launchConnect(const RenderParams& rp, const SceneView& sc, const PathPool& pool, const LaunchConfig& cfg, bool count,
                   hipStream_t stream);
void launchTail(const RenderParams& rp, const SceneView& sc, const PathPool& pool, const EnvLodView& env, const LaunchConfig& cfg, uint32_t* dList,
                uint32_t* dListCount, uint32_t* dListHead, bool count, hipStream_t stream);
void launchResolve(const RenderParams& rp, const PathPool& pool, uint32_t partCount, float* dOut, hipStream_t stream);
void launchResolveCov(const RenderParams& rp, const PathPool& pool, uint32_t partCount, float4* dMean, float* dCov, hipStream_t stream);

void launchTraceRays(const SceneView& sc, const float4* dRays, uint64_t n, bool anyHit, PtrHit* dOut, const LaunchConfig& cfg,
                     uint64_t* dCounters, hipStream_t stream);

void launchAovs(const RenderParams& rp, const SceneView& sc, uint32_t sample, float4* dAlbedo, float4* dNormal, const LaunchConfig& cfg,
                hipStream_t stream);

void launchDebugEvalBsdf(const float4* dMaterial, const RenderParams& rp, const float* dIn, uint64_t n, float* dOut,
                         hipStream_t stream);
void launchDebugSampleBsdf(const float4* dMaterial, const RenderParams& rp, const float* dIn, const uint32_t* dFront,
                           const uint32_t* dRng, uint64_t n, float* dOut, uint32_t* dRngOut, hipStream_t stream);
void launchDebugSampleLobes(const float4* dMaterial, const RenderParams& rp, const float* dIn, const uint32_t* dFront, const uint32_t* dRng,
                            uint64_t n, float* dOut, float* dSample, uint32_t* dRngOut, hipStream_t stream);
void launchDebugEnvLookup(const RenderParams& rp, const SceneView& sc, const EnvLodView& env, const float4* dIn, uint64_t n, float4* dOut,
                          hipStream_t stream);
void launchDebugTexSample(const SceneView& sc, uint32_t texture, const float* dIn, uint64_t n, float4* dOut, hipStream_t stream);
void launchDebugTexSampleGrad(const SceneView& sc, uint32_t texture, const float* dIn, uint64_t n, float4* dOut, hipStream_t stream);
void launchDebugFirstHit(const RenderParams& rp, const SceneView& sc, const uint32_t* dXys, uint64_t n, float* dOut, const LaunchConfig& cfg,
                         hipStream_t stream);
void launchDebugHitRecords(const SceneView& sc, const float4* dRays, const float2* dHits, uint64_t n, uint32_t triCount, uint32_t sphereCount,
                           PtrHit* dOut, hipStream_t stream);
void launchDebugSurfaceHits(const SceneView& sc, const float* dIn, uint64_t n, float* dOut, const LaunchConfig& cfg, hipStream_t stream);
void launchDebugCameraRays(const RenderParams& rp, const uint32_t* dXys, uint64_t n, float* dOut, uint32_t* dRngOut,
                           hipStream_t stream);
void launchDebugEnvSample(const RenderParams& rp, const SceneView& sc, const float* dU, uint64_t n, float4* dOut, hipStream_t stream);
void launchDebugEnvEval(const RenderParams& rp, const SceneView& sc, const float* dDir, uint64_t n, float4* dOut, hipStream_t stream);
void launchDebugRectLightNee(const RenderParams& rp, const SceneView& sc, const PathPool& pool, const float4* dMaterial, const float* dRays,
                             const float* dThr, const uint32_t* dRng, uint64_t n, float4* dHead, uint32_t* dRngOut, const LaunchConfig& cfg,
                             hipStream_t stream);
void launchDebugLightConnection(const RenderParams& rp, const SceneView& sc, const float* dIn, uint64_t n, float* dOut, hipStream_t stream);

}
```

### metal-pathtracer-arm64_amd/csrc/kernels/wavefront.hip

```cpp
#include <hip/hip_runtime.h>

#include <algorithm>

#include "bsdf.h"
#include "device_types.h"
#include "launch.h"
#include <type_traits>
#include "traverse.h"
#include "texture.h"
#include "vec.h"

namespace ptrk {

namespace {

constexpr float kEps = 1.0e-4f;
constexpr float kSpecNeePdfFloor = 1.0e-4f;
constexpr float kSpecNeeInvPdfClamp = 1.0e4f;
constexpr float kMisMin = 1.0e-4f;
constexpr float kMisMax = 0.9999f;
#ifndef PTR_SHADE_BLOCK
#define PTR_SHADE_BLOCK 128
#endif
constexpr uint32_t kShadeBlock = PTR_SHADE_BLOCK;
// ... 997 lines not shown
    uint32_t waveTicks[kShadeParts] = {0u, 0u, 0u, 0u, 0u, 0u, 0u, 0u, 0u, 0u};
};

template <bool COUNT>
__device__ __forceinline__ long long partBegin() { return COUNT ? clock64() : 0ll; }
template <bool COUNT>
__device__ __forceinline__ void partEnd(ShadeCounts& counts, uint32_t part, long long t0) {
    if (COUNT) {
        const uint32_t ticks = static_cast<uint32_t>(clock64() - t0);
        counts.laneTicks[part] += ticks;
        const unsigned long long here = __ballot(true);
        if (laneId() + 1u == static_cast<uint32_t>(__ffsll(static_cast<long long>(here)))) counts.waveTicks[part] += ticks;
    }
}

typedef float NativeFloat4 __attribute__((ext_vector_type(4)));
struct UniformRows {
    const __attribute__((address_space(4))) NativeFloat4* p;
    __device__ __forceinline__ float4 operator[](uint32_t i) const {
        const NativeFloat4 v = p[i];
        return make_float4(v.x, v.y, v.z, v.w);
    }
};
__device__ __forceinline__ UniformRows uniformRows(const float4* p) {
    return UniformRows{reinterpret_cast<const __attribute__((address_space(4))) NativeFloat4*>(reinterpret_cast<uintptr_t>(p))};
}

template <bool COUNT, bool SSS, uint32_t MATS, bool ONE>
__device__ __forceinline__ bool rectLightNee(const RenderParams& rp, const SceneView& sc, const PathPool& pool, uint32_t slot, const Mat& mat,
                                             const Surface& sf, const OffsetFrame& of, f3 n, f3 wo, f3 thr, const ClampCfg& cc, uint32_t depth,
                                             uint32_t& rng, ShadeCounts& counts) {
    const uint32_t nL = ONE ? 1u : sc.rectLightCount;
    const uint32_t sel = min(static_cast<uint32_t>(rngNext(rng) * static_cast<float>(nL)), nL - 1u);
    const float lu = rngNext(rng);
    const float lv = rngNext(rng);
    const float4* Lv = sc.rectLights + static_cast<size_t>(sel) * kRectLightVec4;
    const UniformRows Lu = uniformRows(sc.rectLights);
    auto row = [&](uint32_t i) { return ONE ? Lu[i] : Lv[i]; };
    const float4 l0 = row(0), l1 = row(1), l2 = row(2), l3 = row(3);
    const f3 samplePoint = (mk3(l0) + lu * mk3(l1)) + lv * mk3(l2);
    const f3 toLight = samplePoint - sf.position;
    const float distSq = dot(toLight, toLight);
    if (!(distSq > 0.0f && l0.w > 0.0f)) return false;
    const float distance = sqrtf(distSq);
    const f3 ldir = toLight / distance;
    float cosLight = dot(-ldir, mk3(l3));
    if (l1.w != 0.0f) cosLight = fabsf(cosLight);
    if (!(cosLight > 0.0f)) return false;
    const float pdfArea = 1.0f / l0.w;
    const float pdfDir = pdfArea * distSq / smax(cosLight, 1.0e-6f);
    const float pdf = pdfDir * (1.0f / static_cast<float>(nL));
    const f3 emission = mk3(row(4)) * rp.emissionScale;
    const float nDotL = smax(dot(n, ldir), 0.0f);
    if (!(pdf > 0.0f && isfinite(pdf) && (dot(emission, emission) > 0.0f) && nDotL > 0.0f)) return false;
    if (COUNT) counts.stage[4] += 1u;
    const BsdfEvalResult be = evalBsdf<SSS, MATS>(mat, sf.position, n, wo, ldir, cc);
    if (!neeContributes<SSS>(be, cc)) return false;
    const float w = neeWeight<SSS>(pdf, be.pdf, cc);
    f3 contrib = (emission * be.value) * nDotL;
    contrib *= w / pdf;
    if (!finite3(contrib)) return false;
    const f3 clamped = clampFirefly(thr, contrib, cc);
    if (!(clamped.x > 0.0f || clamped.y > 0.0f || clamped.z > 0.0f)) return false;
    const float shadowMax = smax(distance * (1.0f - rp.shadowSlack) - kEps, kEps);
    const f3 shadowOrg = offsetOrigin(of, ldir);
    float tt, tu, tv;
    bool occludedByLight = false;
    if (COUNT) counts.stage[5] += 1u;
    if (l3.w != 0.0f) {
        occludedByLight = triangleTest(mk3(row(5)), mk3(row(6)), mk3(row(7)), shadowOrg, ldir, kEps, shadowMax, tt, tu, tv) ||
                          triangleTest(mk3(row(8)), mk3(row(9)), mk3(row(10)), shadowOrg, ldir, kEps, shadowMax, tt, tu, tv);
    }
    if (occludedByLight) return false;
    if (COUNT) counts.stage[6] += 1u;
    storeRecord(pool, slot, 0u, 0u, shadowOrg, shadowMax, ldir, clamped, static_cast<float>(depth), mk3(0.0f));
    return true;
}

template <bool SSS>
__device__ __forceinline__ bool surfaceIsDelta(const Mat& mat, uint32_t type, const ClampCfg& cc) {
    bool surfaceDelta = materialIsDelta(mat);
    if (SSS && cc.metalPbr && type == 7u) surfaceDelta = mat.roughness01() <= 1.0e-3f;
    return surfaceDelta;
}

constexpr int kShadeDense = 0, kShadeListed = 1, kShadeTail = 2;
template <bool COUNT, bool SSS, bool TEX, int MODE, uint32_t MATS = kAllMaterials>
__device__ __forceinline__ void shadeSlot(const RenderParams& rp, const SceneView& sc, const PathPool& pool, const uint32_t slot, const bool inRange,
                                          const bool drained, const uint32_t listWave, ShadeCounts& counts, const EnvLodView& env) {
    constexpr bool TAIL = MODE == kShadeTail;
    const long long tLoad = partBegin<COUNT>();
    const uint32_t at = inRange ? slot : 0u;
    float4 ray1v = pool.ray1[at];
    if (!TAIL && drained) {
        const uint32_t peek = __float_as_uint(ray1v.w);
        const bool busy = inRange && (peek & (kFlagAlive | kFlagFlush | (kFlagPendingMask << kFlagPendingShift))) != 0u;
        if (__ballot(busy) == 0ull) return;
    }
    const float4 ray0v = pool.ray0[at];
    uint2 reservation = make_uint2(0u, 0u);
    if (MODE == kShadeDense && (slot & ~63u) < pool.slots) reservation = pool.itemReserve[__builtin_amdgcn_readfirstlane(slot / 64u)];
    const float2 hitv = pool.hit[at];
    const float4 thr4 = pool.thr[at];
    const float4 acc4 = pool.accum[at];
    const uint32_t flagsIn = inRange ? __float_as_uint(ray1v.w) : 0u;
    const uint32_t pendingIn = (flagsIn >> kFlagPendingShift) & kFlagPendingMask;
    constexpr uint32_t kRecords = SSS ? 0x1Fu : shadeRecords(MATS);
    float4 landed[kRecSlots];
#pragma unroll
    for (uint32_t k = 0; k < kRecSlots; ++k) {
        landed[k] = make_float4(0.0f, 0.0f, 0.0f, 0.0f);
        if (kRecords & (1u << k)) {
            const float4* src = (pendingIn & (1u << k)) ? pool.rec[k].a + at : pool.zero;
            landed[k] = *src;
        }
    }
    asm volatile("" ::"v"(acc4.x), "v"(ray0v.x), "v"(hitv.x), "v"(thr4.x));
#pragma unroll
    for (uint32_t k = 0; k < kRecSlots; ++k) {
        if (kRecords & (1u << k)) asm volatile("" ::"v"(landed[k].x));
    }
    const bool active = inRange && (flagsIn & kFlagAlive);
    const bool touched = inRange && (active || pendingIn != 0u || (flagsIn & kFlagFlush));
    if (COUNT) {
        counts.stage[0] += 1u;
        counts.stage[1] += active ? 1u : 0u;
    }

    bool want[kRecSlots] = {false, false, false, false, false};
    bool stillAlive = false, needItem = false, walkFlag = false;
    uint32_t shadedHit = 0u, triHit = 0u, primary = 0u;
    uint32_t rng = __float_as_uint(thr4.w);
    uint32_t item = __float_as_uint(acc4.w);
    uint32_t depth = 0u, specDepth = 0u, mediumDepth = 0u;
    bool lastDelta = true, flushNext = false;
    f3 acc = mk3(0.0f), thr = mk3(1.0f), nextO = mk3(0.0f), nextD = mk3(0.0f);
    float lastPdf = 1.0f;
    uint32_t sig = 0u;
    float2 cone = make_float2(0.0f, 0.0f);
    bool haveCone = false, newSample = false;

    const uint32_t envWidth = (MATS & kFeatureEnvironment) ? sc.envWidth : 0u;
    const bool envSampling = (MATS & kFeatureEnvironment) && sc.envSampling;
    const uint32_t mediaMode = (MATS & kFeatureMedia) ? rp.mediaMode : 0u;
    const bool envLodOn = SSS && env.slotLod != nullptr;
    float envLodNext = -1.0f;

    if (touched) {
        const ClampCfg cc = clampCfg<SSS>(rp);
        acc = mk3(acc4);
#pragma unroll
        for (uint32_t k = 0; k < kRecSlots; ++k) {
            if ((kRecords & (1u << k)) && (pendingIn & (1u << k))) acc += mk3(landed[k]);
        }
        if (COUNT && pool.signature) {
            sig = pool.signature[slot];
            if ((pendingIn & 1u) && (landed[0].x > 0.0f || landed[0].y > 0.0f || landed[0].z > 0.0f)) {
                const uint32_t d = static_cast<uint32_t>(landed[0].w);
                if (d < kSigNeeBits) sig |= 1u << d;
            }
        }
        if (flagsIn & kFlagFlush) {
            pool.itemAccum[pool.flushItem[slot]] = mk4(acc, __uint_as_float(sig));
            acc = mk3(0.0f);
            sig = 0u;
        }
        partEnd<COUNT>(counts, kShadePartLoad, tLoad);

        if (active) {
            depth = (flagsIn >> kFlagDepthShift) & kFlagFieldMask;
            specDepth = (flagsIn >> kFlagSpecDepthShift) & kFlagFieldMask;
            mediumDepth = (flagsIn >> kFlagMediumShift) & 0xFu;
            lastDelta = (flagsIn & kFlagLastDelta) != 0u;
            const f3 rayO = mk3(ray0v);
            const f3 rayD = mk3(ray0v.w, ray1v.x, ray1v.y);
            thr = mk3(thr4);
            lastPdf = ray1v.z;
            const uint32_t prim = __float_as_uint(hitv.y);
            if (COUNT && depth == 0u) primary = 1u;

            bool endPath = false;
            nextO = rayO;
            nextD = rayD;
            bool walking = false;

            if (SSS && (flagsIn & kFlagWalk)) {
                const long long tWalk = partBegin<COUNT>();
                const ShadowRecordView& wr = pool.rec[4];
                const float4 w0 = wr.org[slot], w1 = wr.dir[slot], w2 = wr.a[slot], w3 = wr.b[slot];
                const uint32_t entryMaterial = __float_as_uint(w1.w);
                const Mat mat{sc.materials + static_cast<size_t>(min(entryMaterial, sc.materialCount - 1u)) * kMaterialVec4};
                SssWalk walk{rayO, rayD, mk3(w2), __float_as_uint(w2.w)};
                f3 hitPoint = rayO, outward = mk3(0.0f);
                if (prim != kHitMiss) {
                    const Surface bsf = reconstruct(sc, rayO, rayD, hitv.x, prim);
                    hitPoint = bsf.position;
                    outward = bsf.normal;
                }
                BsdfSampleResult bs{mk3(0.0f), mk3(0.0f), 0.0f, false, 0, false, mk3(0.0f)};
                int outcome = sssWalkStep(mat, rp.sssMaxSteps, walk, prim != kHitMiss, hitv.x, hitPoint, outward, rng, bs);
                if (outcome == kWalkWalking) {
                    walking = true;
                    nextO = walk.position;
                    nextD = walk.direction;
                    wr.a[slot] = mk4(walk.throughput, __uint_as_float(walk.step));
                } else {
                    const f3 entryN = mk3(w3);
                    if (outcome == kWalkFallback) bs = sampleBsdf<true>(mat, mk3(w0), entryN, entryN, -entryN, true, rng, cc);
                    if (bs.pdf <= 0.0f || dot(bs.dir, bs.dir) <= 0.0f || !finite3(bs.weight)) {
                        endPath = true;
                    } else {
                        specDepth = 0u;
                        thr *= bs.weight;
                        thr = clampThroughput(thr, cc);
                        const float maxComp = smax(smax(thr.x, thr.y), thr.z);
                        if (!finite3(thr) || maxComp <= 0.0f) {
                            endPath = true;
                        } else {
                            lastPdf = bs.pdf > 0.0f ? bs.pdf : lastPdf;
                            lastDelta = false;
                            if (outcome == kWalkSample) {
                                nextO = sssExitOrigin(bs.exitPoint, outward, bs.dir);
                            } else {
                                const f3 on = mk3(w1);
                                const float sign = dot(bs.dir, on) >= 0.0f ? 1.0f : -1.0f;
                                nextO = mk3(w0) + on * (sign * smax(fabsf(w0.w) * 1.0e-4f, kEps));
                                nextO += (bs.dir * kEps) * 0.5f;
                            }
                            nextD = bs.dir;
                            if (rp.enableRussianRoulette && depth >= 5u) {
                                const float p = clampf(maxComp, 0.05f, 0.95f);
                                if (rngNext(rng) > p) {
                                    endPath = true;
                                } else {
                                    thr /= p;
                                }
                            }
                        }
                    }
                }
                partEnd<COUNT>(counts, kShadePartWalk, tWalk);
            } else if (prim == kHitMiss) {
                const long long tMiss = partBegin<COUNT>();
                f3 bg;
                if (rp.backgroundMode == PTR_BG_SOLID) {
                    bg = ld3(rp.backgroundColor);
                } else if (rp.backgroundMode == PTR_BG_ENVIRONMENT && envWidth > 0u) {
                    const float lod = (envLodOn && depth > 0u) ? env.slotLod[slot] : -1.0f;
                    bg = lod >= 0.0f ? envLookupLod(sc, env, rayD, rp.envRotation, rp.envIntensity, lod) : envLookup(sc, rayD, rp.envRotation, rp.envIntensity);
                } else {
                    bg = skyColor(rayD);
                }
                float mis = 1.0f;
                const bool useMis = (!lastDelta) || rp.enableSpecularNee || rp.enableMnee;
                if (useMis && envSampling) mis = bsdfSideMis(lastPdf, envPdfOf(sc, rayD, rp.envRotation));
                acc += clampFirefly(thr, bg * mis, cc);
                if (COUNT) sig = (sig & 0xFFFFu) | (sigHashStep(sig >> 16, 7u, 0u, 0u) << 16);
                endPath = true;
                partEnd<COUNT>(counts, kShadePartMiss, tMiss);
            } else if (sc.materialCount == 0u) {
                endPath = true;
            } else {
                const long long tSurface = partBegin<COUNT>();
                const Surface sf = reconstruct(sc, rayO, rayD, hitv.x, prim);
                const OffsetFrame of = offsetFrame(sf);
                if (COUNT) {
                    shadedHit = 1u;
                    if (COUNT) counts.stage[2] += 1u;
                    triHit = sf.primType == 0u ? 1u : 0u;
                    sig = (sig & 0xFFFFu) | (sigHashStep(sig >> 16, sf.primType, sf.geomIndex, sf.primIndex) << 16);
                }
                if ((mediaMode & PTR_METAL_MEDIA) && mediumDepth > 0u) {
                    const uint32_t inside = mediumEntry(pool.medium[slot], mediumDepth - 1u);
                    const Mat mm{sc.materials + static_cast<size_t>(min(inside, sc.materialCount - 1u)) * kMaterialVec4};
                    const f3 sigma = mm.sigmaA();
                    if (sigma.x > 0.0f || sigma.y > 0.0f || sigma.z > 0.0f) {
                        const float segment = smax(hitv.x, 0.0f);
                        thr *= mk3(expf(-sigma.x * segment), expf(-sigma.y * segment), expf(-sigma.z * segment));
                    }
                }
                const uint32_t materialIndex = min(sf.material, sc.materialCount - 1u);
                Mat mat{byteOffset(sc.materials, materialIndex * (kMaterialVec4 * 16u))};
                const uint32_t type = mat.type();
                const f3 incident = normalize(rayD);
                const f3 wo = -incident;
                f3 n = sf.hitShadingNormal;
                if (dot(n, n) <= 0.0f) n = sf.normal;
                if (type == 2u) {
                    n = sf.normal;
                    if ((mediaMode & PTR_METAL_FACE_NORMAL) && !sf.frontFace) n = -n;
                }
                n = normalize(n);
                bool hitTwoSided = sf.twoSided;
                bool passThrough = false;
                PbrHit pbrHit;
                if (SSS && cc.metalPbr && type == 7u) {
                    if (TEX && sf.primType == 0u && sc.textureCount > 0u && sc.triUv != nullptr) {
                        cone = pool.cone ? pool.cone[slot] : make_float2(0.0f, 0.0f);
                        haveCone = pool.cone != nullptr;
                        if ((rp.mediaMode & PTR_METAL_RAY_DIFF) && depth == 0u) {
                            passThrough = applyPbrTextures<true>(sc, sf, materialIndex, mat, wo, cone, hitv.x, firstHitUvGrads(rp, sc, sf, rayD, hitv.x),
                                                                 rng, pbrHit);
                        } else {
                            passThrough = applyPbrTextures<false>(sc, sf, materialIndex, mat, wo, cone, hitv.x, noUvGrads(), rng, pbrHit);
                        }
                        if (!passThrough) {
                            mat.o = pbrHit.ov;
                            n = pbrHit.shadingNormal;
                            hitTwoSided = pbrHit.twoSided;
                        }
                    }
                    if (!passThrough) {
                        const f3 emission = mk3(mat.v(kMatEmission));
                        if ((emission.x != 0.0f || emission.y != 0.0f || emission.z != 0.0f) && (sf.frontFace || hitTwoSided)) {
                            acc += clampFirefly(thr, emission, cc);
                        }
                    }
                }

                partEnd<COUNT>(counts, kShadePartSurface, tSurface);
                if (SSS && passThrough) {
                    nextO = offsetOrigin(of, rayD);
                    nextD = rayD;
                    lastPdf = 1.0f;
                    lastDelta = true;
                    specDepth += 1u;
                } else if (type == 3u) {
                    const long long tEmitter = partBegin<COUNT>();
                    if (COUNT) counts.stage[3] += 1u;
                    const float4 em = mat.v(kMatEmission);
                    f3 emission = mk3(em) * rp.emissionScale;
                    if (em.w > 0.0f && envWidth > 0u && sf.frontFace) {
                        emission *= envLookup(sc, -n, rp.envRotation, rp.envIntensity);
                    }
                    if ((dot(emission, emission) > 0.0f) && (sf.frontFace || sf.twoSided)) {
                        float mis = 1.0f;
                        const bool useMis = (!lastDelta) || rp.enableSpecularNee || rp.enableMnee;
                        if (useMis && sc.rectLightCount > 0u) {
                            mis = bsdfSideMis(lastPdf, rectLightPdfForHit(sc, sf.primType, sf.primIndex, sf.position, rayO));
// ... 546 lines not shown
                    if (COUNT) ++raysExtend;
                    const TraceHit h = traverse<false, COUNT>(sc, mk3(r0), mk3(r0.w, r1.x, r1.y), kEps, INFINITY, stack, cntExtend);
                    pool.hit[slot] = make_float2(h.t, __uint_as_float(h.prim));
                    __threadfence();
                }
                shadeSlot<COUNT, SSS, TEX, kShadeTail>(rp, sc, pool, slot, true, false, 0u, counts, env);
                __threadfence();
                uint32_t bits = (__float_as_uint(pool.ray1[slot].w) >> kFlagPendingShift) & kFlagPendingMask;
                while (bits != 0u) {
                    const uint32_t rec = static_cast<uint32_t>(__ffs(static_cast<int>(bits))) - 1u;
                    bits &= bits - 1u;
                    const uint32_t recAt = rec * 4u * slots + slot;
                    const float4 o4 = recBase[recAt], d4 = recBase[recAt + slots];
                    float4* const a = recBase + recAt + 2u * slots;
                    const uint32_t kind = __float_as_uint(d4.w);
                    if (kind == 0u || kind == 3u) {
                        if (COUNT) ++raysAny;
                        const uint32_t ignore = kind == 3u ? __float_as_uint(recBase[recAt + 3u * slots].x) : kHitMiss;
                        const TraceHit h = traverse<true, COUNT>(sc, mk3(o4), mk3(d4), kEps, o4.w, stack, cntAny, ignore);
                        if (COUNT) early += anyHitFound(h.prim) ? 1u : 0u;
                        if (anyHitFound(h.prim)) *a = make_float4(0.0f, 0.0f, 0.0f, 0.0f);
                    } else if (kind == 1u) {
                        if (COUNT) ++raysClosest;
                        const TraceHit h = traverse<false, COUNT>(sc, mk3(o4), mk3(d4), kEps, INFINITY, stack, cntClosest);
                        const float4 a4 = *a;
                        const f3 c = rectContribution(rp, sc, cc, mk3(o4), mk3(d4), h, mk3(a4), a4.w, mk3(recBase[recAt + 3u * slots]));
                        *a = mk4(c, 0.0f);
                    } else {
                        const float4 a4 = *a;
                        const f3 c = mneeChain<COUNT>(rp, sc, cc, mk3(o4), mk3(d4), __float_as_uint(o4.w), mk3(a4), a4.w, mk3(recBase[recAt + 3u * slots]),
                                                      stack, cntAny, cntClosest, raysAny, raysClosest);
                        *a = mk4(c, 0.0f);
                    }
                }
                __threadfence();
            }
        }
    }
    addTraceCounters<COUNT>(pool.counters, raysAny, cntAny, raysExtend + raysClosest,
                            TraceCounters{cntExtend.nodes + cntClosest.nodes, cntExtend.prims + cntClosest.prims});
    if (COUNT) {
        addCounter(pool.counters, kCntShadowEarlyExit, early);
        addCounter(pool.counters, kCntShadedHits, counts.shadedHit);
        addCounter(pool.counters, kCntTriangleHits, counts.triHit);
        addCounter(pool.counters, kCntPrimaryRays, counts.primary);
        addCounter(pool.counters, kCntExtendRays, counts.settled);
    }
}

__global__ void __launch_bounds__(256) k_flush(RenderParams rp, PathPool pool) {
    const uint32_t slot = blockIdx.x * blockDim.x + threadIdx.x;
    if (slot >= pool.slots) return;
    const uint32_t flags = __float_as_uint(pool.ray1[slot].w);
    if (!(flags & kFlagFlush)) return;
    const uint32_t pendingIn = (flags >> kFlagPendingShift) & kFlagPendingMask;
    f3 acc = mk3(pool.accum[slot]);
    uint32_t sig = pool.signature ? pool.signature[slot] : 0u;
    for (uint32_t k = 0; k < kRecSlots; ++k) {
        if (!(pendingIn & (1u << k))) continue;
        const float4 a = pool.rec[k].a[slot];
        acc += mk3(a);
        if (k == 0u && (a.x > 0.0f || a.y > 0.0f || a.z > 0.0f) && static_cast<uint32_t>(a.w) < kSigNeeBits) sig |= 1u << static_cast<uint32_t>(a.w);
    }
    pool.itemAccum[pool.flushItem[slot]] = mk4(acc, __uint_as_float(sig));
    (void)rp;
}

__global__ void __launch_bounds__(256) k_resolve(RenderParams rp, PathPool pool, uint32_t partCount, float* out) {
    const uint32_t lp = blockIdx.x * blockDim.x + threadIdx.x;
    if (lp >= rp.localPixels) return;
    f3 sum = mk3(0.0f);
    for (uint32_t c = 0; c < rp.spp; ++c) sum += mk3(pool.itemAccum[static_cast<size_t>(c) * rp.localPixels + lp]);
    const uint32_t pixel = pool.pixelOfLocal[lp];
    const uint32_t x = pixel % rp.width, y = pixel / rp.width;
    const uint32_t localBand = (y / PTR_BAND_ROWS) / partCount;
    float* o = out + (static_cast<size_t>(localBand * PTR_BAND_ROWS + (y % PTR_BAND_ROWS)) * rp.width + x) * 3u;
    f3 total = (rp.passFlags & 1u) ? sum : mk3(o[0], o[1], o[2]) + sum;
    if (rp.passFlags & 2u) total = total / static_cast<float>(rp.sppTotal);
    o[0] = total.x;
    o[1] = total.y;
    o[2] = total.z;
}

__global__ void __launch_bounds__(kTraceBlock) k_aovs(RenderParams rp, SceneView sc, uint32_t sample, float4* albedo, float4* normal, uint32_t* spill,
                                                       uint32_t spillStride) {
    __shared__ uint32_t ldsStack[kLdsStackLevels * kTraceBlock];
    const uint32_t gtid = blockIdx.x * kTraceBlock + threadIdx.x;
    LaneStack stack = laneStack(ldsStack, spill, spillStride, sc);
    TraceCounters cnt{0u, 0u};
    const uint32_t pixels = rp.width * rp.height;
    for (uint32_t pixel = gtid; pixel < pixels; pixel += gridDim.x * kTraceBlock) {
        uint32_t rng;
        f3 org, dir;
        beginSample(rp, pixel, sample, rng, org, dir);
        const TraceHit h = traverse<false, false>(sc, org, dir, kEps, INFINITY, stack, cnt);
        float4 a = make_float4(0.0f, 0.0f, 0.0f, 0.0f), n = make_float4(0.5f, 0.5f, 0.5f, 0.0f);
        if (h.prim != kHitMiss && sc.materialCount > 0u) {
            const Surface sf = reconstruct(sc, org, dir, h.t, h.prim);
            const Mat mat{sc.materials + static_cast<size_t>(min(sf.material, sc.materialCount - 1u)) * kMaterialVec4};
            f3 sn = sf.hitShadingNormal;
            if (dot(sn, sn) <= 0.0f) sn = sf.normal;
            if (mat.type() == 2u) sn = sf.normal;
            sn = normalize(sn);
            a = mk4(mat.baseColor(), 1.0f);
            n = mk4(sn * 0.5f + mk3(0.5f), h.t);
        }
        albedo[pixel] = a;
        normal[pixel] = n;
    }
}

__device__ __forceinline__ PtrHit ptrHitOf(const SceneView& sc, f3 org, f3 dir, const TraceHit& h, bool anyHit) {
    float hu = 0.0f, hv = 0.0f;
    PtrHit r;
    r.t = -1.0f;
    r.u = 0.0f;
    r.v = 0.0f;
    r.primType = 0u;
    r.geomIndex = 0u;
    r.primIndex = 0u;
    r.ng[0] = r.ng[1] = r.ng[2] = 0.0f;
    r.pad = 0u;
    if (h.prim != kHitMiss) {
        r.t = anyHit ? 0.0f : h.t;
        if (!anyHit) {
            if (h.prim & kHitSphereBit) {
                r.primType = 1u;
                r.primIndex = sc.sphereInfo[h.prim & kHitIndexMask].x;
            } else {
                const float4* tp = sc.tris + static_cast<size_t>(h.prim & kHitIndexMask) * 3u;
                const float4 t0 = tp[0], t1 = tp[1], t2 = tp[2];
                const uint32_t meta = __float_as_uint(t1.w);
                triangleUv(mk3(t0), mk3(t1), mk3(t2), org, dir, hu, hv);
                r.u = hu;
                r.v = hv;
                const f3 ng = cross(mk3(t2), mk3(t1));
                r.ng[0] = ng.x;
                r.ng[1] = ng.y;
                r.ng[2] = ng.z;
                if ((meta >> 30) == 0u) {
                    r.primType = 0u;
                    r.geomIndex = meta & kTriGeomMask;
                    r.primIndex = __float_as_uint(t2.w);
                } else {
                    r.primType = 2u;
                    r.primIndex = meta & kTriGeomMask;
                }
            }
        }
    }
    return r;
}

template <bool ANY>
__global__ void __launch_bounds__(kTraceBlock) k_trace_rays(SceneView sc, const float4* rays, uint64_t n, PtrHit* out, uint32_t* spill,
                                                             uint32_t spillStride, uint64_t* counters) {
    __shared__ uint32_t ldsStack[kLdsStackLevels * kTraceBlock];
    const uint32_t gtid = blockIdx.x * kTraceBlock + threadIdx.x;
    LaneStack stack = laneStack(ldsStack, spill, spillStride, sc);
    TraceCounters cnt{0u, 0u};
    for (uint64_t i = gtid; i < n; i += static_cast<uint64_t>(gridDim.x) * kTraceBlock) {
        const float4 a = rays[i * 2u], b = rays[i * 2u + 1u];
        const f3 org = mk3(a), dir = mk3(b);
        const TraceHit h = traverse<ANY, true>(sc, org, dir, a.w, b.w, stack, cnt);
        out[i] = ptrHitOf(sc, org, dir, h, ANY);
    }
// ... 319 lines not shown
        withBools([&](auto aliveTag) {
            hipLaunchKernelGGL((k_extend<decltype(countTag)::value, decltype(aliveTag)::value, decltype(nodesTag)::value>), dim3(t.grid), dim3(kTraceBlock),
                               0, stream, sc, pool, t.cfg.spill, t.stride, t.cfg.workCounters, t.cfg.refillBelow, t.cfg.feederChunk, aliveOut);
        }, aliveOut != nullptr);
    });
}

constexpr uint32_t kMetalInstantiationBits = PTR_METAL_SSS | PTR_METAL_PBR | PTR_METAL_CLAMPS | PTR_METAL_ENV_LOD;
struct ShadeVariant {
    bool sss;
    bool tex;
    uint32_t set;
};
static ShadeVariant shadeVariant(const RenderParams& rp, const SceneView& sc, bool count) {
    ShadeVariant v;
    v.sss = (rp.mediaMode & kMetalInstantiationBits) != 0u;
    v.tex = v.sss && sc.textureCount > 0u;
    v.set = kAllMaterials;
    if (v.sss || count || sc.materialTypes == 0u) return v;
    const uint32_t needs = sc.materialTypes | ((sc.envWidth > 0u || sc.envSampling) ? kFeatureEnvironment : 0u) |
                           ((rp.mediaMode & (PTR_METAL_MEDIA | PTR_METAL_FACE_NORMAL)) ? kFeatureMedia : 0u);
    for (uint32_t set : {kDiffuseMaterials, kBasicMaterials, kMetalMaterials, kCarPaintMaterials, kPbrMaterials}) {
        if ((needs & ~set) == 0u) {
            v.set = set;
            break;
        }
    }
    return v;
}

uint32_t shadeKernelSet(const RenderParams& rp, const SceneView& sc, bool count) { return shadeVariant(rp, sc, count).set; }

void launchShade(const RenderParams& rp, const SceneView& sc, const PathPool& pool, const ShadeResets& resets, const EnvLodView& env, bool count,
                 hipStream_t stream) {
    const ShadeVariant v = shadeVariant(rp, sc, count);
    const bool listed = pool.busyIn != nullptr;
    const uint32_t grid = ceilDiv(pool.slots, kShadeBlock);
    auto launch = [&](auto kernel) { hipLaunchKernelGGL(kernel, dim3(grid), dim3(kShadeBlock), 0, stream, rp, sc, pool, resets, env); };
    withBools([&](auto countTag, auto listedTag) {
        constexpr bool C = decltype(countTag)::value, L = decltype(listedTag)::value;
        if (v.tex) launch(k_shade<C, true, true, L>);
        else if (v.sss) launch(k_shade<C, true, false, L>);
        else if (C) launch(k_shade<C, false, false, L>);
        else if (v.set == kDiffuseMaterials) launch(k_shade<false, false, false, L, kDiffuseMaterials>);
        else if (v.set == kBasicMaterials) launch(k_shade<false, false, false, L, kBasicMaterials>);
        else if (v.set == kMetalMaterials) launch(k_shade<false, false, false, L, kMetalMaterials>);
        else if (v.set == kCarPaintMaterials) launch(k_shade<false, false, false, L, kCarPaintMaterials>);
        else if (v.set == kPbrMaterials) launch(k_shade<false, false, false, L, kPbrMaterials>);
        else launch(k_shade<C, false, false, L>);
    }, count, listed);
}

void launchConnect(const RenderParams& rp, const SceneView& sc, const PathPool& pool, const LaunchConfig& cfgIn, bool count, hipStream_t stream) {
    const TraceLaunch t = traceLaunch(cfgIn);
    withNodeFormat(sc, count, [&](auto countTag, auto nodesTag) {
        hipLaunchKernelGGL((k_connect<decltype(countTag)::value, decltype(nodesTag)::value>), dim3(t.grid), dim3(kTraceBlock), 0, stream, rp, sc, pool,
                           t.cfg.spill, t.stride, t.cfg.workCounters + 1, t.cfg.refillBelow, t.cfg.feederChunk);
    });
    if (rp.enableMnee && rp.enableMneeSecondary) {
        withBools([&](auto countTag) {
            hipLaunchKernelGGL(k_connect_chain<decltype(countTag)::value>, dim3(t.grid), dim3(kTraceBlock), 0, stream, rp, sc, pool, t.cfg.spill, t.stride);
        }, count);
    }
}

void launchTail(const RenderParams& rp, const SceneView& sc, const PathPool& pool, const EnvLodView& env, const LaunchConfig& cfgIn, uint32_t* dList,
                uint32_t* dListCount, uint32_t* dListHead, bool count, hipStream_t stream) {
    const TraceLaunch t = traceLaunch(cfgIn);
    const uint32_t collectGrid = std::max(1u, std::min(t.grid, ceilDiv(pool.slots, 256u * 16u)));
    hipLaunchKernelGGL(k_tail_collect, dim3(collectGrid), dim3(256), 0, stream, pool, dList, dListCount);
    const ShadeVariant v = shadeVariant(rp, sc, count);
    withBools([&](auto countTag, auto sssTag, auto texTag) {
        constexpr bool C = decltype(countTag)::value, S = decltype(sssTag)::value, T = decltype(texTag)::value;
        hipLaunchKernelGGL((k_tail_run<C, S, S && T>), dim3(t.grid), dim3(kTraceBlock), 0, stream, rp, sc, pool, dList, dListCount, dListHead,
                           t.cfg.spill, t.stride, env);
    }, count, v.sss, v.tex);
}

void launchResolve(const RenderParams& rp, const PathPool& pool, uint32_t partCount, float* dOut, hipStream_t stream) {
    hipLaunchKernelGGL(k_flush, dim3(ceilDiv(pool.slots, 256)), dim3(256), 0, stream, rp, pool);
    hipLaunchKernelGGL(k_resolve, dim3(ceilDiv(rp.localPixels, 256)), dim3(256), 0, stream, rp, pool, partCount, dOut);
}

void launchTraceRays(const SceneView& sc, const float4* dRays, uint64_t n, bool anyHit, PtrHit* dOut, const LaunchConfig& cfgIn,
                     uint64_t* dCounters, hipStream_t stream) {
    const TraceLaunch t = traceLaunch(cfgIn, n);
    withBools([&](auto anyTag) {
        hipLaunchKernelGGL(k_trace_rays<decltype(anyTag)::value>, dim3(t.grid), dim3(kTraceBlock), 0, stream, sc, dRays, n, dOut, t.cfg.spill, t.stride,
                           dCounters);
    }, anyHit);
}

void launchAovs(const RenderParams& rp, const SceneView& sc, uint32_t sample, float4* dAlbedo, float4* dNormal, const LaunchConfig& cfgIn,
                hipStream_t stream) {
    const TraceLaunch t = traceLaunch(cfgIn, rp.width * rp.height);
    hipLaunchKernelGGL(k_aovs, dim3(t.grid), dim3(kTraceBlock), 0, stream, rp, sc, sample, dAlbedo, dNormal, t.cfg.spill, t.stride);
}

void launchDebugEvalBsdf(const float4* dMaterial, const RenderParams& rp, const float* dIn, uint64_t n, float* dOut, hipStream_t stream) {
    launchFlat(k_debug_eval, 128, n, stream, dMaterial, rp, dIn, n, dOut);
}

void launchDebugSampleBsdf(const float4* dMaterial, const RenderParams& rp, const float* dIn, const uint32_t* dFront, const uint32_t* dRng,
                           uint64_t n, float* dOut, uint32_t* dRngOut, hipStream_t stream) {
    launchFlat(k_debug_sample, 128, n, stream, dMaterial, rp, dIn, dFront, dRng, n, dOut, dRngOut);
}

void launchDebugSampleLobes(const float4* dMaterial, const RenderParams& rp, const float* dIn, const uint32_t* dFront, const uint32_t* dRng,
                            uint64_t n, float* dOut, float* dSample, uint32_t* dRngOut, hipStream_t stream) {
    launchFlat(k_debug_sample_lobes, 128, n, stream, dMaterial, rp, dIn, dFront, dRng, n, dOut, dSample, dRngOut);
}

void launchDebugEnvLookup(const RenderParams& rp, const SceneView& sc, const EnvLodView& env, const float4* dIn, uint64_t n, float4* dOut,
                          hipStream_t stream) {
    launchFlat(k_debug_env_lookup, 128, n, stream, rp, sc, env, dIn, n, dOut);
}

void launchDebugTexSample(const SceneView& sc, uint32_t texture, const float* dIn, uint64_t n, float4* dOut, hipStream_t stream) {
    launchFlat(k_debug_tex_sample, 128, n, stream, sc, texture, dIn, n, dOut);
}

void launchDebugTexSampleGrad(const SceneView& sc, uint32_t texture, const float* dIn, uint64_t n, float4* dOut, hipStream_t stream) {
    launchFlat(k_debug_tex_sample_grad, 128, n, stream, sc, texture, dIn, n, dOut);
}

void launchDebugFirstHit(const RenderParams& rp, const SceneView& sc, const uint32_t* dXys, uint64_t n, float* dOut, const LaunchConfig& cfgIn,
                         hipStream_t stream) {
    const TraceLaunch t = traceLaunch(cfgIn, n);
    hipLaunchKernelGGL(k_debug_first_hit, dim3(t.grid), dim3(kTraceBlock), 0, stream, rp, sc, dXys, n, dOut, t.cfg.spill, t.stride);
}

void launchDebugHitRecords(const SceneView& sc, const float4* dRays, const float2* dHits, uint64_t n, uint32_t triCount, uint32_t sphereCount,
                           PtrHit* dOut, hipStream_t stream) {
    launchFlat(k_debug_hit_records, 256, n, stream, sc, dRays, dHits, n, triCount, sphereCount, dOut);
}

void launchDebugSurfaceHits(const SceneView& sc, const float* dIn, uint64_t n, float* dOut, const LaunchConfig& cfgIn, hipStream_t stream) {
    const TraceLaunch t = traceLaunch(cfgIn, n);
    hipLaunchKernelGGL(k_debug_surface, dim3(t.grid), dim3(kTraceBlock), 0, stream, sc, dIn, n, dOut, t.cfg.spill, t.stride);
}

void launchDebugCameraRays(const RenderParams& rp, const uint32_t* dXys, uint64_t n, float* dOut, uint32_t* dRngOut, hipStream_t stream) {
    launchFlat(k_debug_camera, 128, n, stream, rp, dXys, n, dOut, dRngOut);
}

void launchDebugEnvSample(const RenderParams& rp, const SceneView& sc, const float* dU, uint64_t n, float4* dOut, hipStream_t stream) {
    launchFlat(k_debug_env_sample, 128, n, stream, rp, sc, dU, n, dOut);
}

void launchDebugEnvEval(const RenderParams& rp, const SceneView& sc, const float* dDir, uint64_t n, float4* dOut, hipStream_t stream) {
    launchFlat(k_debug_env_eval, 128, n, stream, rp, sc, dDir, n, dOut);
}

void launchDebugRectLightNee(const RenderParams& rp, const SceneView& sc, const PathPool& pool, const float4* dMaterial, const float* dRays,
                             const float* dThr, const uint32_t* dRng, uint64_t n, float4* dHead, uint32_t* dRngOut, const LaunchConfig& cfgIn,
                             hipStream_t stream) {
    const TraceLaunch t = traceLaunch(cfgIn, n);
    withBools([&](auto oneTag, auto sssTag) {
        hipLaunchKernelGGL((k_debug_rect_light_nee<decltype(sssTag)::value, decltype(oneTag)::value>), dim3(t.grid), dim3(kTraceBlock), 0, stream, rp, sc,
                           pool, dMaterial, dRays, dThr, dRng, n, dHead, dRngOut, t.cfg.spill, t.stride);
    }, sc.rectLightCount == 1u, shadeVariant(rp, sc, false).sss);
}

void launchDebugLightConnection(const RenderParams& rp, const SceneView& sc, const float* dIn, uint64_t n, float* dOut, hipStream_t stream) {
    launchFlat(k_debug_light_connection, 128, n, stream, rp, sc, shadeVariant(rp, sc, false).sss, dIn, n, dOut);
}
// ... 3 lines not shown
```

Measured before the change: 2616 Msamples/s.

## Cull camera pixels whose primary rays cannot hit scene bounds and shade them directly

Computes world bounds of all primitives at upload, or from the root box for dynamic scenes. It projects that box, padded for lens radius, onto the image plane to get a conservative screen rectangle. Pixels outside the rectangle skip the wavefront path pool. A lightweight k_background kernel evaluates their escaped radiance (sky, solid colour or environment, with MIS) for every sample and writes the band output directly. This removes primary traversal and wavefront scheduling for pixels that can only see background. It adds host-side geometry checks and an extra kernel launch, and falls back to no culling for degenerate cameras, a camera inside the bounds, covariance passes or stats modes.

```diff
diff --git a/include/ptr_background.h b/include/ptr_background.h
--- /dev/null
+++ b/include/ptr_background.h
@@ -0,0 +1,16 @@
+#ifndef PTR_BACKGROUND_H
+#define PTR_BACKGROUND_H
+
+#include "ptr_abi.h"
+
+#ifdef __cplusplus
+extern "C" {
+#endif
+
+int ptr_background_debug_cull(const PtrDeviceScene* scene, const PtrSceneDesc* desc, const PtrSettings* settings, uint32_t part, uint32_t parts,
+                              int count, uint32_t out[8], double bounds[7], char* err, size_t err_cap);
+
+#ifdef __cplusplus
+}
+#endif
+#endif
diff --git a/metal-pathtracer-arm64_amd/__init__.py b/metal-pathtracer-arm64_amd/__init__.py
--- a/metal-pathtracer-arm64_amd/__init__.py
+++ b/metal-pathtracer-arm64_amd/__init__.py
@@ -452,6 +452,11 @@
 }
 DYNAMIC_SYMBOLS = tuple(_DYNAMIC_SIGNATURES)
 
+_BACKGROUND_SIGNATURES = {
+    "ptr_background_debug_cull": (_int, [_vp, _desc, _settings, _u32, _u32, _int, _up, C.POINTER(C.c_double)] + _err),
+}
+BACKGROUND_SYMBOLS = tuple(_BACKGROUND_SIGNATURES)
+
 SCENE_ARRAYS = {"tris": (0, np.float32, (3, 4)), "triNormals": (1, np.float32, (3, 4)), "triUv": (2, np.float32, (4, 4)),
                 "triTangent": (3, np.float32, (3, 4)), "triBounds": (4, np.float32, (2, 4)), "sphereBounds": (5, np.float32, (2, 4)),
                 "boxes": (6, np.float32, (4, 4)), "qnodes": (7, np.uint32, (2, 4)), "wnodes": (8, np.uint32, (4, 4)), "grid": (9, np.float32, (3,))}
@@ -479,7 +484,7 @@
     lib = C.CDLL(path)
     for name, (restype, argtypes) in list(_SIGNATURES.items()) + list(_POST_SIGNATURES.items()) + list(_STATS_SIGNATURES.items()) + \
             list(_ADAPTIVE_SIGNATURES.items()) + list(_MULTI_SIGNATURES.items()) + list(_FRAME_SIGNATURES.items()) + list(_MULTI_FRAME_SIGNATURES.items()) + \
-            list(_DYNAMIC_SIGNATURES.items()):
+            list(_DYNAMIC_SIGNATURES.items()) + list(_BACKGROUND_SIGNATURES.items()):
         fn = getattr(lib, name)
         fn.restype, fn.argtypes = restype, argtypes
     _lib = lib
@@ -1323,6 +1328,17 @@
                    "spheres", "sah_cost_milli", "build_ms", "quantized_usable")
 
 
+def background_cull(settings: PtrSettings, scene: Optional["DeviceScene"] = None, desc: Optional[PtrSceneDesc] = None, part: int = 0,
+                    parts: int = 1, count: bool = False) -> dict:
+    out = (C.c_uint32 * 8)()
+    bounds = (C.c_double * 7)()
+    err = _err_buf()
+    _check(load_library().ptr_background_debug_cull(scene._h if scene is not None else None, C.byref(desc) if desc is not None else None,
+                                                    C.byref(settings), part, parts, int(count), out, bounds, err, len(err)), err)
+    return {"culling": bool(out[0]), "rect": (int(out[1]), int(out[2]), int(out[3]), int(out[4])), "traced": int(out[5]),
+            "background": int(out[6]), "lo": np.array(bounds[0:3]), "hi": np.array(bounds[3:6]), "bounds_valid": bool(bounds[6])}
+
+
 def debug_scene_geometry(desc: PtrSceneDesc, leaf_max: int = 0) -> dict:
     out = (C.c_uint64 * 16)()
     err = _err_buf()
diff --git a/metal-pathtracer-arm64_amd/csrc/host/background_cull.cpp b/metal-pathtracer-arm64_amd/csrc/host/background_cull.cpp
--- /dev/null
+++ b/metal-pathtracer-arm64_amd/csrc/host/background_cull.cpp
@@ -0,0 +1,121 @@
+#include "background_cull.h"
+
+#include <algorithm>
+#include <cmath>
+
+namespace ptr {
+
+namespace {
+
+struct D3 {
+    double x, y, z;
+};
+D3 operator+(D3 a, D3 b) { return {a.x + b.x, a.y + b.y, a.z + b.z}; }
+D3 operator-(D3 a, D3 b) { return {a.x - b.x, a.y - b.y, a.z - b.z}; }
+D3 operator*(double s, D3 a) { return {s * a.x, s * a.y, s * a.z}; }
+double dot(D3 a, D3 b) { return a.x * b.x + a.y * b.y + a.z * b.z; }
+D3 cross(D3 a, D3 b) { return {a.y * b.z - a.z * b.y, a.z * b.x - a.x * b.z, a.x * b.y - a.y * b.x}; }
+D3 ld(const float* p) { return {p[0], p[1], p[2]}; }
+bool finite(D3 a) { return std::isfinite(a.x) && std::isfinite(a.y) && std::isfinite(a.z); }
+
+}
+
+void WorldBounds::add(const double p[3], double pad) {
+    for (int a = 0; a < 3; ++a) {
+        lo[a] = valid ? std::min(lo[a], p[a] - pad) : p[a] - pad;
+        hi[a] = valid ? std::max(hi[a], p[a] + pad) : p[a] + pad;
+    }
+    valid = true;
+}
+
+WorldBounds boundsOfPrimitives(const float* triData, uint64_t triCount, const float* sphereData, uint64_t sphereCount) {
+    WorldBounds b;
+    for (uint64_t i = 0; i < triCount; ++i) {
+        const float* t = triData + i * 12u;
+        const double v0[3] = {t[0], t[1], t[2]};
+        const double v1[3] = {v0[0] - t[4], v0[1] - t[5], v0[2] - t[6]};
+        const double v2[3] = {v0[0] + t[8], v0[1] + t[9], v0[2] + t[10]};
+        b.add(v0);
+        b.add(v1);
+        b.add(v2);
+    }
+    for (uint64_t i = 0; i < sphereCount; ++i) {
+        const float* s = sphereData + i * 4u;
+        const double c[3] = {s[0], s[1], s[2]};
+        b.add(c, std::fabs(static_cast<double>(s[3])));
+    }
+    if (!b.valid) return b;
+    double scale = 0.0;
+    for (int a = 0; a < 3; ++a) scale = std::max(scale, std::max(std::fabs(b.lo[a]), std::fabs(b.hi[a])));
+    const double pad = scale * 1.0e-5 + 1.0e-30;
+    for (int a = 0; a < 3; ++a) {
+        b.lo[a] -= pad;
+        b.hi[a] += pad;
+        if (!std::isfinite(b.lo[a]) || !std::isfinite(b.hi[a])) b.valid = false;
+    }
+    return b;
+}
+
+CullRect backgroundCullRect(const CullCamera& cam, uint32_t width, uint32_t height, const WorldBounds& bounds) {
+    const CullRect none;
+    if (!bounds.valid || width == 0u || height == 0u) return none;
+    const D3 origin = ld(cam.origin), lowerLeft = ld(cam.lowerLeft), horizontal = ld(cam.horizontal), vertical = ld(cam.vertical);
+    const double lens = cam.lensRadius > 0.0f ? static_cast<double>(cam.lensRadius) : 0.0;
+    if (!finite(origin) || !finite(lowerLeft) || !finite(horizontal) || !finite(vertical) || !std::isfinite(cam.lensRadius)) return none;
+    const double hh = dot(horizontal, horizontal), vv = dot(vertical, vertical);
+    D3 axis = cross(horizontal, vertical);
+    const double axisLength = std::sqrt(dot(axis, axis));
+    if (!(hh > 0.0) || !(vv > 0.0) || !(axisLength > 0.0) || !std::isfinite(axisLength)) return none;
+    axis = (1.0 / axisLength) * axis;
+    if (std::fabs(dot(horizontal, vertical)) > 1.0e-5 * std::sqrt(hh * vv)) return none;
+    const D3 centre = (lowerLeft + 0.5 * horizontal) + 0.5 * vertical;
+    double planeDepth = dot(axis, centre - origin);
+    if (planeDepth < 0.0) {
+        axis = -1.0 * axis;
+        planeDepth = -planeDepth;
+    }
+    if (!(planeDepth > 0.0) || !std::isfinite(planeDepth)) return none;
+    if (lens > 0.0) {
+        const D3 lu = ld(cam.u), lv = ld(cam.v);
+        if (!finite(lu) || !finite(lv)) return none;
+        if (std::fabs(dot(axis, lu)) > 1.0e-5 * std::sqrt(dot(lu, lu)) || std::fabs(dot(axis, lv)) > 1.0e-5 * std::sqrt(dot(lv, lv))) return none;
+    }
+
+    double lo[3], hi[3];
+    for (int a = 0; a < 3; ++a) {
+        lo[a] = bounds.lo[a] - lens;
+        hi[a] = bounds.hi[a] + lens;
+        if (!std::isfinite(lo[a]) || !std::isfinite(hi[a]) || lo[a] > hi[a]) return none;
+    }
+    const double o[3] = {origin.x, origin.y, origin.z};
+    if (o[0] >= lo[0] && o[0] <= hi[0] && o[1] >= lo[1] && o[1] <= hi[1] && o[2] >= lo[2] && o[2] <= hi[2]) return none;
+
+    double uMin = INFINITY, uMax = -INFINITY, vMin = INFINITY, vMax = -INFINITY;
+    for (int k = 0; k < 8; ++k) {
+        const D3 corner{(k & 1) ? hi[0] : lo[0], (k & 2) ? hi[1] : lo[1], (k & 4) ? hi[2] : lo[2]};
+        const D3 q = corner - origin;
+        const double depth = dot(axis, q);
+        if (!(depth > lens) || !(depth > 0.0)) return none;
+        const D3 onPlane = origin + (planeDepth / depth) * q;
+        const D3 rel = onPlane - lowerLeft;
+        const double u = dot(rel, horizontal) / hh, v = dot(rel, vertical) / vv;
+        if (!std::isfinite(u) || !std::isfinite(v)) return none;
+        uMin = std::min(uMin, u), uMax = std::max(uMax, u);
+        vMin = std::min(vMin, v), vMax = std::max(vMax, v);
+    }
+    const double uPad = lens / std::sqrt(hh), vPad = lens / std::sqrt(vv);
+    const double xLo = (uMin - uPad) * width, xHi = (uMax + uPad) * width;
+    const double yLo = (1.0 - (vMax + vPad)) * height, yHi = (1.0 - (vMin - vPad)) * height;
+    if (!std::isfinite(xLo) || !std::isfinite(xHi) || !std::isfinite(yLo) || !std::isfinite(yHi)) return none;
+    auto firstPixel = [](double at, uint32_t n) { return static_cast<uint32_t>(std::min(std::max(std::floor(at) - 1.0, 0.0), static_cast<double>(n))); };
+    auto endPixel = [](double at, uint32_t n) { return static_cast<uint32_t>(std::min(std::max(std::floor(at) + 2.0, 0.0), static_cast<double>(n))); };
+    CullRect r;
+    r.x0 = firstPixel(xLo, width), r.x1 = endPixel(xHi, width);
+    r.y0 = firstPixel(yLo, height), r.y1 = endPixel(yHi, height);
+    if (r.x0 >= r.x1 || r.y0 >= r.y1) r.x0 = r.x1 = r.y0 = r.y1 = 0u;
+    if (r.x0 == 0u && r.y0 == 0u && r.x1 == width && r.y1 == height) return none;
+    r.cull = true;
+    return r;
+}
+
+}
diff --git a/metal-pathtracer-arm64_amd/csrc/host/background_cull.h b/metal-pathtracer-arm64_amd/csrc/host/background_cull.h
--- /dev/null
+++ b/metal-pathtracer-arm64_amd/csrc/host/background_cull.h
@@ -0,0 +1,29 @@
+#pragma once
+
+#include <cstdint>
+
+namespace ptr {
+
+struct CullCamera {
+    const float *origin, *lowerLeft, *horizontal, *vertical, *u, *v;
+    float lensRadius;
+};
+
+struct WorldBounds {
+    double lo[3] = {0.0, 0.0, 0.0}, hi[3] = {0.0, 0.0, 0.0};
+    bool valid = false;
+    void add(const double p[3], double pad = 0.0);
+};
+
+WorldBounds boundsOfPrimitives(const float* triData, uint64_t triCount, const float* sphereData, uint64_t sphereCount);
+
+struct CullRect {
+    bool cull = false;
+    uint32_t x0 = 0, x1 = 0, y0 = 0, y1 = 0;
+    bool inside(uint32_t x, uint32_t y) const { return x >= x0 && x < x1 && y >= y0 && y < y1; }
+    bool operator==(const CullRect& o) const { return cull == o.cull && x0 == o.x0 && x1 == o.x1 && y0 == o.y0 && y1 == o.y1; }
+};
+
+CullRect backgroundCullRect(const CullCamera& cam, uint32_t width, uint32_t height, const WorldBounds& bounds);
+
+}
diff --git a/metal-pathtracer-arm64_amd/csrc/host/debug_probes.cpp b/metal-pathtracer-arm64_amd/csrc/host/debug_probes.cpp
--- a/metal-pathtracer-arm64_amd/csrc/host/debug_probes.cpp
+++ b/metal-pathtracer-arm64_amd/csrc/host/debug_probes.cpp
@@ -2,6 +2,7 @@
 #include <cmath>
 
 #include "device_scene.h"
+#include "ptr_background.h"
 #include "ptr_debug.h"
 
 using namespace ptrk;
@@ -237,6 +238,36 @@
             occluded[i] = (a.x == 0.0f && a.y == 0.0f && a.z == 0.0f) ? 1u : 0u;
         }
     });
+}
+
+int ptr_background_debug_cull(const PtrDeviceScene* scene, const PtrSceneDesc* desc, const PtrSettings* settings, uint32_t part, uint32_t parts,
+                              int count, uint32_t out[8], double bounds[7], char* err, size_t err_cap) {
+    const char* who = "ptr_background_debug_cull";
+    if ((!scene && !desc) || !settings || !out) return nullArgument(who, err, err_cap);
+    if (parts == 0u || part >= parts) return refuse(err, err_cap, std::string(who) + ": bad partition");
+    try {
+        ptr::WorldBounds world;
+        if (scene) {
+            world = scene->worldBounds;
+        } else {
+            ptr::PreparedGeometry pg;
+            prepareGeometry(*desc, pg);
+            world = ptr::boundsOfPrimitives(pg.geo.triData.data(), pg.geo.triData.size() / 12u, pg.geo.sphereData.data(), pg.geo.sphereData.size() / 4u);
+        }
+        const ptr::CullRect rect = passCullRect(world, *settings, false, count != 0 ? 1 : 0);
+        std::vector<uint32_t> pixels;
+        partitionPixels(settings->width, settings->height, part, parts, pixels);
+        uint32_t traced = 0u;
+        for (const uint32_t pixel : pixels) traced += (!rect.cull || rect.inside(pixel % settings->width, pixel / settings->width)) ? 1u : 0u;
+        const uint32_t words[8] = {rect.cull ? 1u : 0u, rect.x0, rect.x1, rect.y0, rect.y1, traced, static_cast<uint32_t>(pixels.size()) - traced, 0u};
+        std::copy(words, words + 8, out);
+        if (bounds) {
+            for (int a = 0; a < 3; ++a) bounds[a] = world.lo[a], bounds[3 + a] = world.hi[a];
+            bounds[6] = world.valid ? 1.0 : 0.0;
+        }
+        return 0;
+    }
+    PTR_CATCH_ALL(err, err_cap)
 }
 
 int ptr_debug_exact_division(uint32_t d, const uint32_t* n, uint64_t count, uint32_t* out) {
diff --git a/metal-pathtracer-arm64_amd/csrc/host/device_scene.h b/metal-pathtracer-arm64_amd/csrc/host/device_scene.h
--- a/metal-pathtracer-arm64_amd/csrc/host/device_scene.h
+++ b/metal-pathtracer-arm64_amd/csrc/host/device_scene.h
@@ -12,6 +12,7 @@
 
 #include "../kernels/device_types.h"
 #include "../kernels/launch.h"
+#include "background_cull.h"
 #include "env_importance_sampler.h"
 #include "geometry_cache.h"
 #include "ptr_abi.h"
@@ -169,7 +170,10 @@
     uint32_t* pinnedAlive = nullptr;
     uint32_t traceGrid = 0;
     uint32_t traceGridHalf = 0;
-    uint32_t cachedW = 0, cachedH = 0, cachedPart = 0, cachedParts = 0, cachedLocalPixels = 0;
+    uint32_t cachedW = 0, cachedH = 0, cachedPart = 0, cachedParts = 0, cachedLocalPixels = 0, cachedBackgroundPixels = 0;
+    ptr::CullRect cachedCull;
+    DeviceBuffer<uint32_t> backgroundPixels;
+    ptr::WorldBounds worldBounds;
 
     ~PtrDeviceScene() {
         if (pinnedAlive) (void)hipHostFree(pinnedAlive);
@@ -187,6 +191,7 @@
 double ensureEnvMips(PtrDeviceScene& ds);
 void fillRenderParams(const PtrSettings& s, uint32_t spp, ptrk::RenderParams& rp);
 ptrk::LaunchConfig coldLaunchConfig(const PtrDeviceScene& ds);
+ptr::CullRect passCullRect(const ptr::WorldBounds& world, const PtrSettings& settings, bool covariance, int mode);
 void renderBands(PtrDeviceScene& ds, const PtrSettings& settings, uint32_t spp, uint32_t part, uint32_t parts, float* dOut, hipStream_t stream,
                  int mode, PtrRenderStats* stats, float* dCov = nullptr);
 uint32_t framePasses(const PtrDeviceScene& ds, const PtrSettings& settings, uint32_t spp);
diff --git a/metal-pathtracer-arm64_amd/csrc/host/dynamic.cpp b/metal-pathtracer-arm64_amd/csrc/host/dynamic.cpp
--- a/metal-pathtracer-arm64_amd/csrc/host/dynamic.cpp
+++ b/metal-pathtracer-arm64_amd/csrc/host/dynamic.cpp
@@ -149,6 +149,11 @@
                     v.gridInvCell[a] = 1.0f / v.gridCell[a];
                 }
             }
+        }
+        ds.worldBounds = ptr::WorldBounds{};
+        if (dyn.nodeCount > 0u && v.oversizeRef == kRefEmpty && rootBoxOf(dyn.rootBox, lo, hi)) {
+            for (int a = 0; a < 3; ++a) ds.worldBounds.lo[a] = lo[a], ds.worldBounds.hi[a] = hi[a];
+            ds.worldBounds.valid = true;
         }
         if (v.useQuantized) launchDynQuantise(boxes, ds.qnodes.ptr, dyn.nodeCount, v.gridOrigin, v.gridCell, st);
         HIP_CHECK(hipEventRecord(dyn.events[3], st));
diff --git a/metal-pathtracer-arm64_amd/csrc/host/hip_backend.cpp b/metal-pathtracer-arm64_amd/csrc/host/hip_backend.cpp
--- a/metal-pathtracer-arm64_amd/csrc/host/hip_backend.cpp
+++ b/metal-pathtracer-arm64_amd/csrc/host/hip_backend.cpp
@@ -290,6 +290,8 @@
         v.materialTex = ds.materialTex.ptr;
         v.textureCount = desc.textureCount;
     }
+
+    ds.worldBounds = ptr::boundsOfPrimitives(geo.triData.data(), geo.triData.size() / 12u, geo.sphereData.data(), geo.sphereData.size() / 4u);
 
     if (ps.dynamic) uploadDynamicTables(ps, ds);
 
@@ -474,6 +476,16 @@
             }
         }
     }
+}
+
+ptr::CullRect passCullRect(const ptr::WorldBounds& world, const PtrSettings& settings, bool covariance, int mode) {
+    if (!ptr::readKnobs().backgroundCull || covariance || (mode & 5) != 0 || settings.width == 0u || settings.height == 0u) return ptr::CullRect{};
+    RenderParams rp;
+    fillRenderParams(settings, 1u, rp);
+    if (rp.maxDepth == 0u) return ptr::CullRect{};
+    const CameraParams& c = rp.cam;
+    return ptr::backgroundCullRect(ptr::CullCamera{c.origin, c.lowerLeft, c.horizontal, c.vertical, c.u, c.v, c.lensRadius}, settings.width,
+                                   settings.height, world);
 }
 
 void addLaunchStats(PtrRenderStats& a, const PtrRenderStats& b) {
@@ -714,7 +726,7 @@
     return r;
 }
 
-enum class SpanKind : int { Extend = 0, Shade = 1, Connect = 2, Tail = 3, ResolveCov = 4 };
+enum class SpanKind : int { Extend = 0, Shade = 1, Connect = 2, Tail = 3, ResolveCov = 4, Background = 5 };
 
 struct LaunchTimer {
     struct Span {
@@ -769,6 +781,7 @@
             case SpanKind::Connect: stats.shadowKernelMs += ms; break;
             case SpanKind::Tail: stats.tailKernelMs += ms; break;
             case SpanKind::ResolveCov: break;
+            case SpanKind::Background: break;
         }
     }
     if (!count) return;
@@ -815,29 +828,66 @@
                  100.0 * static_cast<double>(c[kCntExtendRefillTicks]) / std::max(static_cast<double>(c[kCntExtendWaveTicks]), 1.0));
 }
 
+struct BackgroundPixels {
+    const uint32_t* pixels = nullptr;
+    uint32_t count = 0, parts = 1;
+    float* out = nullptr;
+};
+
 template <typename Resolve>
 void tracePass(PtrDeviceScene& ds, const PtrSettings& settings, uint32_t spp, uint32_t sampleBase, uint32_t sppTotal, uint32_t passFlags,
-               const uint32_t* dPixelOfLocal, uint32_t localPixels, hipStream_t stream, int mode, PtrRenderStats* stats, Resolve&& resolve);
+               const uint32_t* dPixelOfLocal, uint32_t localPixels, hipStream_t stream, int mode, PtrRenderStats* stats, Resolve&& resolve,
+               const BackgroundPixels& background = BackgroundPixels{});
 
 void renderPass(PtrDeviceScene& ds, const PtrSettings& settings, uint32_t spp, uint32_t sampleBase, uint32_t sppTotal, uint32_t passFlags,
                 uint32_t part, uint32_t parts, float* dOut, float* dCov, hipStream_t stream, int mode, PtrRenderStats* stats) {
-    if (ds.cachedW != settings.width || ds.cachedH != settings.height || ds.cachedPart != part || ds.cachedParts != parts) {
-        std::vector<uint32_t> pixels;
+    const ptr::CullRect cull = ptrhost::passCullRect(ds.worldBounds, settings, dCov != nullptr, mode);
+    if (ds.cachedW != settings.width || ds.cachedH != settings.height || ds.cachedPart != part || ds.cachedParts != parts || !(ds.cachedCull == cull)) {
+        std::vector<uint32_t> pixels, background;
         partitionPixels(settings.width, settings.height, part, parts, pixels);
+        if (cull.cull) {
+            size_t kept = 0;
+            for (const uint32_t pixel : pixels) {
+                if (cull.inside(pixel % settings.width, pixel / settings.width)) pixels[kept++] = pixel;
+                else background.push_back(pixel);
+            }
+            pixels.resize(kept);
+        }
         ds.pixelOfLocal.upload(pixels.data(), pixels.size());
+        ds.backgroundPixels.upload(background.data(), background.size());
         ds.cachedW = settings.width;
         ds.cachedH = settings.height;
         ds.cachedPart = part;
         ds.cachedParts = parts;
+        ds.cachedCull = cull;
         ds.cachedLocalPixels = static_cast<uint32_t>(pixels.size());
+        ds.cachedBackgroundPixels = static_cast<uint32_t>(background.size());
     }
     const uint32_t localPixels = ds.cachedLocalPixels;
+    const BackgroundPixels background{ds.backgroundPixels.ptr, ds.cachedBackgroundPixels, parts, dOut};
     const uint32_t bandCount = ptr_part_band_count(settings.height, part, parts);
     const size_t outFloats = static_cast<size_t>(bandCount) * PTR_BAND_ROWS * settings.width * 3u;
     if (passFlags & 1u) HIP_CHECK(hipMemsetAsync(dOut, 0, outFloats * sizeof(float), stream));
     if (dCov && (passFlags & 1u)) HIP_CHECK(hipMemsetAsync(dCov, 0, outFloats * 2u * sizeof(float), stream));
     if (localPixels == 0) {
+        const auto wall0 = std::chrono::steady_clock::now();
+        if (background.count > 0u) {
+            RenderParams rp;
+            fillRenderParams(settings, spp, rp);
+            rp.sampleBase = sampleBase;
+            rp.sppTotal = std::max(1u, sppTotal);
+            rp.passFlags = passFlags;
+            launchBackground(rp, ds.view, background.pixels, background.count, parts, dOut, stream);
+            HIP_CHECK(hipGetLastError());
+        }
         HIP_CHECK(hipStreamSynchronize(stream));
+        if (stats && background.count > 0u) {
+            std::memset(stats, 0, sizeof(*stats));
+            stats->totalSeconds = std::chrono::duration<double>(std::chrono::steady_clock::now() - wall0).count();
+            stats->avgMsPerSample = stats->totalSeconds * 1000.0 / std::max(1u, spp);
+            stats->uploadSeconds = ds.uploadSeconds;
+            stats->samples = static_cast<uint64_t>(background.count) * std::max(1u, spp);
+        }
         return;
     }
     tracePass(ds, settings, spp, sampleBase, sppTotal, passFlags, ds.pixelOfLocal.ptr, localPixels, stream, mode, stats,
@@ -847,12 +897,15 @@
                       ds.covMean.ensure(localPixels);
                       timer.launch(SpanKind::ResolveCov, stream, [&] { launchResolveCov(rp, pool, parts, ds.covMean.ptr, dCov, stream); });
                   }
-              });
+              },
+              background);
+    if (stats) stats->samples += static_cast<uint64_t>(background.count) * std::max(1u, spp);
 }
 
 template <typename Resolve>
 void tracePass(PtrDeviceScene& ds, const PtrSettings& settings, uint32_t spp, uint32_t sampleBase, uint32_t sppTotal, uint32_t passFlags,
-               const uint32_t* dPixelOfLocal, uint32_t localPixels, hipStream_t stream, int mode, PtrRenderStats* stats, Resolve&& resolve) {
+               const uint32_t* dPixelOfLocal, uint32_t localPixels, hipStream_t stream, int mode, PtrRenderStats* stats, Resolve&& resolve,
+               const BackgroundPixels& background) {
     const bool count = (mode & 1) != 0;
     const bool soloGroup = (mode & 2) != 0;
 
@@ -899,6 +952,10 @@
     HIP_CHECK(hipGetLastError());
     HIP_CHECK(hipEventRecord(ds.groupEvents[0], stream));
     for (size_t g = 1; g < groups.size(); ++g) HIP_CHECK(hipStreamWaitEvent(groups[g].stream, ds.groupEvents[0], 0));
+    if (background.count > 0u) {
+        timer.launch(SpanKind::Background, stream,
+                     [&] { launchBackground(rp, ds.view, background.pixels, background.count, background.parts, background.out, stream); });
+    }
     uint64_t iterations = 0;
     const uint64_t perBounce = ((rp.mediaMode & PTR_METAL_SSS) && rp.sssMode == 2u && ds.hasRandomWalkMaterial) ? 1ull + rp.sssMaxSteps : 1ull;
     const uint64_t maxIterations = static_cast<uint64_t>(rp.maxDepth) * perBounce * ((itemCount64 + slots - 1) / slots + 1) + 8;
diff --git a/metal-pathtracer-arm64_amd/csrc/host/knobs.cpp b/metal-pathtracer-arm64_amd/csrc/host/knobs.cpp
--- a/metal-pathtracer-arm64_amd/csrc/host/knobs.cpp
+++ b/metal-pathtracer-arm64_amd/csrc/host/knobs.cpp
@@ -44,6 +44,7 @@
     k.refillBelow = static_cast<int>(std::min<long long>(std::max<long long>(numberOr("PTR_REFILL_BELOW", 0), 0), 64));
     k.buildThreads = static_cast<uint32_t>(std::min<long long>(std::max<long long>(numberOr("PTR_BUILD_THREADS", 0), 0), 256));
     k.noOversize = numberOr("PTR_NO_OVERSIZE", 0) != 0;
+    k.backgroundCull = numberOr("PTR_BACKGROUND_CULL", 1) != 0;
     k.denoiseTiled = static_cast<int>(numberOr("PTR_DENOISE_TILED", -1));
     const char* verbose = std::getenv("PTR_VERBOSE");
     k.verboseBuild = hasTopic(verbose, "build");
diff --git a/metal-pathtracer-arm64_amd/csrc/host/knobs.h b/metal-pathtracer-arm64_amd/csrc/host/knobs.h
--- a/metal-pathtracer-arm64_amd/csrc/host/knobs.h
+++ b/metal-pathtracer-arm64_amd/csrc/host/knobs.h
@@ -15,6 +15,7 @@
     int refillBelow = 0;
     uint32_t buildThreads = 0;
     bool noOversize = false;
+    bool backgroundCull = true;
     int denoiseTiled = -1;
     bool verboseBuild = false, verbosePolls = false, verboseLaunches = false, verboseSteps = false;
 };
diff --git a/metal-pathtracer-arm64_amd/csrc/host/stats.cpp b/metal-pathtracer-arm64_amd/csrc/host/stats.cpp
--- a/metal-pathtracer-arm64_amd/csrc/host/stats.cpp
+++ b/metal-pathtracer-arm64_amd/csrc/host/stats.cpp
@@ -71,7 +71,7 @@
         if (framePasses(*scene, *settings, spp) > 1u) throw HipError{"ptr_stats_debug_samples: the frame needs more than one pass"};
         const size_t pixels = static_cast<size_t>(settings->width) * settings->height;
         scene->outBands.ensure(bandPixels(*settings, 0u, 1u) * 3u);
-        renderBands(*scene, *settings, spp, 0u, 1u, scene->outBands.ptr, nullptr, 0, nullptr);
+        renderBands(*scene, *settings, spp, 0u, 1u, scene->outBands.ptr, nullptr, 4, nullptr);
         std::vector<float4> items(pixels * spp);
         std::vector<uint32_t> pixelOfLocal(pixels);
         scene->itemAccum.download(items.data(), items.size());
diff --git a/metal-pathtracer-arm64_amd/csrc/kernels/launch.h b/metal-pathtracer-arm64_amd/csrc/kernels/launch.h
--- a/metal-pathtracer-arm64_amd/csrc/kernels/launch.h
+++ b/metal-pathtracer-arm64_amd/csrc/kernels/launch.h
@@ -32,6 +32,8 @@
 void launchTail(const RenderParams& rp, const SceneView& sc, const PathPool& pool, const EnvLodView& env, const LaunchConfig& cfg, uint32_t* dList,
                 uint32_t* dListCount, uint32_t* dListHead, bool count, hipStream_t stream);
 void launchResolve(const RenderParams& rp, const PathPool& pool, uint32_t partCount, float* dOut, hipStream_t stream);
+void launchBackground(const RenderParams& rp, const SceneView& sc, const uint32_t* dPixels, uint32_t pixelCount, uint32_t partCount, float* dOut,
+                      hipStream_t stream);
 void launchResolveCov(const RenderParams& rp, const PathPool& pool, uint32_t partCount, float4* dMean, float* dCov, hipStream_t stream);
 
 void launchTraceRays(const SceneView& sc, const float4* dRays, uint64_t n, bool anyHit, PtrHit* dOut, const LaunchConfig& cfg,
diff --git a/metal-pathtracer-arm64_amd/csrc/kernels/wavefront.hip b/metal-pathtracer-arm64_amd/csrc/kernels/wavefront.hip
--- a/metal-pathtracer-arm64_amd/csrc/kernels/wavefront.hip
+++ b/metal-pathtracer-arm64_amd/csrc/kernels/wavefront.hip
@@ -1103,6 +1103,25 @@
     bool surfaceDelta = materialIsDelta(mat);
     if (SSS && cc.metalPbr && type == 7u) surfaceDelta = mat.roughness01() <= 1.0e-3f;
     return surfaceDelta;
+}
+
+__device__ __forceinline__ void addEscapedRadiance(const RenderParams& rp, const SceneView& sc, const EnvLodView& env, const ClampCfg& cc, const f3& rayD, const f3& thr,
+                                                   const bool lastDelta, const float lastPdf, const bool storedLod, const uint32_t slot, const uint32_t envWidth,
+                                                   const bool envSampling,
+                                                   f3& acc) {
+    f3 bg;
+    if (rp.backgroundMode == PTR_BG_SOLID) {
+        bg = ld3(rp.backgroundColor);
+    } else if (rp.backgroundMode == PTR_BG_ENVIRONMENT && envWidth > 0u) {
+        const float lod = storedLod ? env.slotLod[slot] : -1.0f;
+        bg = lod >= 0.0f ? envLookupLod(sc, env, rayD, rp.envRotation, rp.envIntensity, lod) : envLookup(sc, rayD, rp.envRotation, rp.envIntensity);
+    } else {
+        bg = skyColor(rayD);
+    }
+    float mis = 1.0f;
+    const bool useMis = (!lastDelta) || rp.enableSpecularNee || rp.enableMnee;
+    if (useMis && envSampling) mis = bsdfSideMis(lastPdf, envPdfOf(sc, rayD, rp.envRotation));
+    acc += clampFirefly(thr, bg * mis, cc);
 }
 
 constexpr int kShadeDense = 0, kShadeListed = 1, kShadeTail = 2;
@@ -1263,19 +1282,7 @@
                 partEnd<COUNT>(counts, kShadePartWalk, tWalk);
             } else if (prim == kHitMiss) {
                 const long long tMiss = partBegin<COUNT>();
-                f3 bg;
-                if (rp.backgroundMode == PTR_BG_SOLID) {
-                    bg = ld3(rp.backgroundColor);
-                } else if (rp.backgroundMode == PTR_BG_ENVIRONMENT && envWidth > 0u) {
-                    const float lod = (envLodOn && depth > 0u) ? env.slotLod[slot] : -1.0f;
-                    bg = lod >= 0.0f ? envLookupLod(sc, env, rayD, rp.envRotation, rp.envIntensity, lod) : envLookup(sc, rayD, rp.envRotation, rp.envIntensity);
-                } else {
-                    bg = skyColor(rayD);
-                }
-                float mis = 1.0f;
-                const bool useMis = (!lastDelta) || rp.enableSpecularNee || rp.enableMnee;
-                if (useMis && envSampling) mis = bsdfSideMis(lastPdf, envPdfOf(sc, rayD, rp.envRotation));
-                acc += clampFirefly(thr, bg * mis, cc);
+                addEscapedRadiance(rp, sc, env, cc, rayD, thr, lastDelta, lastPdf, envLodOn && depth > 0u, slot, envWidth, envSampling, acc);
                 if (COUNT) sig = (sig & 0xFFFFu) | (sigHashStep(sig >> 16, 7u, 0u, 0u) << 16);
                 endPath = true;
                 partEnd<COUNT>(counts, kShadePartMiss, tMiss);
@@ -1988,6 +1995,33 @@
     o[2] = total.z;
 }
 
+template <bool SSS>
+__global__ void __launch_bounds__(256) k_background(RenderParams rp, SceneView sc, const uint32_t* pixels, uint32_t pixelCount, uint32_t partCount,
+                                                    float* out) {
+    const uint32_t i = blockIdx.x * blockDim.x + threadIdx.x;
+    if (i >= pixelCount) return;
+    const uint32_t pixel = pixels[i];
+    const ClampCfg cc = clampCfg<SSS>(rp);
+    const EnvLodView noLod{};
+    f3 sum = mk3(0.0f);
+    for (uint32_t s = 0; s < rp.spp; ++s) {
+        uint32_t rng;
+        f3 org, dir;
+        beginSample(rp, pixel, s, rng, org, dir);
+        f3 value = mk3(0.0f);
+        addEscapedRadiance(rp, sc, noLod, cc, dir, mk3(1.0f), true, 1.0f, false, 0u, sc.envWidth, sc.envSampling != 0u, value);
+        sum += value;
+    }
+    const uint32_t x = pixel % rp.width, y = pixel / rp.width;
+    const uint32_t localBand = (y / PTR_BAND_ROWS) / partCount;
+    float* o = out + (static_cast<size_t>(localBand * PTR_BAND_ROWS + (y % PTR_BAND_ROWS)) * rp.width + x) * 3u;
+    f3 total = (rp.passFlags & 1u) ? sum : mk3(o[0], o[1], o[2]) + sum;
+    if (rp.passFlags & 2u) total = total / static_cast<float>(rp.sppTotal);
+    o[0] = total.x;
+    o[1] = total.y;
+    o[2] = total.z;
+}
+
 __global__ void __launch_bounds__(kTraceBlock) k_aovs(RenderParams rp, SceneView sc, uint32_t sample, float4* albedo, float4* normal, uint32_t* spill,
                                                        uint32_t spillStride) {
     __shared__ uint32_t ldsStack[kLdsStackLevels * kTraceBlock];
@@ -2473,6 +2507,15 @@
     hipLaunchKernelGGL(k_resolve, dim3(ceilDiv(rp.localPixels, 256)), dim3(256), 0, stream, rp, pool, partCount, dOut);
 }
 
+void launchBackground(const RenderParams& rp, const SceneView& sc, const uint32_t* dPixels, uint32_t pixelCount, uint32_t partCount, float* dOut,
+                      hipStream_t stream) {
+    if (pixelCount == 0u) return;
+    withBools([&](auto sssTag) {
+        hipLaunchKernelGGL(k_background<decltype(sssTag)::value>, dim3(ceilDiv(pixelCount, 256)), dim3(256), 0, stream, rp, sc, dPixels, pixelCount,
+                           partCount, dOut);
+    }, shadeVariant(rp, sc, false).sss);
+}
+
 void launchTraceRays(const SceneView& sc, const float4* dRays, uint64_t n, bool anyHit, PtrHit* dOut, const LaunchConfig& cfgIn,
                      uint64_t* dCounters, hipStream_t stream) {
     const TraceLaunch t = traceLaunch(cfgIn, n);
```

Result: faster. 2801 Msamples/s (median of 6 runs) (+7.1%).
